# NVIDIA/audio-flamingo

Hardware: AMD Instinct MI355X
Metric: audio-sec/s + decoder tokens/s, AF3-7B bf16 train (higher is better)
Workload: dtype bf16; 1 GPU; AF3 (AF-Whisper 32L + Qwen2.5-7B 28L, MLP projector) bf16 train step fwd+bwd+AdamW, 30 s clips, S=1024; micro_batch_per_gpu=8, global_batch=8, seq_len=1024, parallelism=dp1, activation_checkpointing=False

## Files before the change

### audio-flamingo_amd/csrc/ceiling.hip

```cpp
#include "common.h"
#include "../../include/afk.h"

namespace {

constexpr int SEG = 16;

template <int MODE>
__global__ __launch_bounds__(512, 1) void mfma_ceiling_kernel(const bf16* __restrict__ src, float* __restrict__ sink, int iters) {
    extern __shared__ __attribute__((aligned(16))) char smem[];
    const int tid = threadIdx.x, lane = tid & 63, wave = tid >> 6;
    bf16x8 a[2][4], b[2][4];
    const bf16x8* s8 = (const bf16x8*)src;
#pragma unroll
    for (int i = 0; i < 2; ++i)
#pragma unroll
        for (int k = 0; k < 4; ++k) {
            a[i][k] = s8[((blockIdx.x * 8 + wave) * 16 + i * 4 + k) * 64 % 8192 + lane];
            b[i][k] = s8[((blockIdx.x * 8 + wave) * 16 + 8 + i * 4 + k) * 64 % 8192 + lane];
        }
    if (MODE == 1) {
        for (int i = tid; i < 4096; i += 512) ((bf16x8*)smem)[i] = s8[i];
        __syncthreads();
    }
    f32x16 acc[2][2];
#pragma unroll
    for (int i = 0; i < 2; ++i)
#pragma unroll
        for (int j = 0; j < 2; ++j)
#pragma unroll
            for (int e = 0; e < 16; ++e) acc[i][j][e] = 0.f;
    uint32_t lds = afk_lds_addr(smem) + lane * 16;
    for (int it = 0; it < iters; ++it) {
        if (MODE == 1) {
            const uint32_t base = lds + ((it * 12 * 1024) & 0xffff & ~0x3fff);
            afk_static_for<4>([&](auto K) {
                constexpr int k = decltype(K)::value;
                a[0][k] = afk_lds_b128<k * 1024>(base);
                a[1][k] = afk_lds_b128<(4 + k) * 1024>(base);
                b[k & 1][k] = afk_lds_b128<(8 + k) * 1024>(base);
            });
            afk_lds_wait0(a[0][0], a[0][1], a[0][2], a[0][3], a[1][0], a[1][1], a[1][2], a[1][3], b[0][0], b[1][1], b[0][2], b[1][3]);
        }
#pragma unroll
        for (int k = 0; k < 4; ++k)
#pragma unroll
            for (int i = 0; i < 2; ++i)
#pragma unroll
                for (int j = 0; j < 2; ++j) acc[i][j] = __builtin_amdgcn_mfma_f32_32x32x16_bf16(a[i][k], b[j][k], acc[i][j], 0, 0, 0);
    }
    float s = 0.f;
#pragma unroll
    for (int i = 0; i < 2; ++i)
#pragma unroll
        for (int j = 0; j < 2; ++j)
#pragma unroll
            for (int e = 0; e < 16; ++e) s += acc[i][j][e];
    if (s == 123.456f) sink[0] = s;
}

template <bool CHAIN>
__global__ __launch_bounds__(256, 1) void mfma_pacing_kernel(const bf16* __restrict__ src, float* __restrict__ sink, int iters) {
    const int lane = threadIdx.x & 63, wave = threadIdx.x >> 6;
    const bf16x8* s8 = (const bf16x8*)src;
    bf16x8 a[4], b[4];
#pragma unroll
    for (int k = 0; k < 4; ++k) {
        a[k] = s8[(wave * 8 + k) * 64 + lane];
        b[k] = s8[(wave * 8 + 4 + k) * 64 + lane];
    }
    f32x16 acc[4];
#pragma unroll
    for (int i = 0; i < 4; ++i)
#pragma unroll
        for (int e = 0; e < 16; ++e) acc[i][e] = 0.f;
    uint64_t t0, t1;
    asm volatile("s_waitcnt vmcnt(0)\n s_memtime %0\n s_waitcnt lgkmcnt(0)" : "=s"(t0)::"memory");
    for (int it = 0; it < iters; ++it) {
        if (CHAIN) {
#pragma unroll
            for (int i = 0; i < 4; ++i)
#pragma unroll
                for (int k = 0; k < 4; ++k) acc[i] = __builtin_amdgcn_mfma_f32_32x32x16_bf16(a[k], b[k], acc[i], 0, 0, 0);
        } else {
#pragma unroll
            for (int k = 0; k < 4; ++k)
#pragma unroll
                for (int i = 0; i < 4; ++i) acc[i] = __builtin_amdgcn_mfma_f32_32x32x16_bf16(a[k], b[k], acc[i], 0, 0, 0);
        }
    }
    float s = 0.f;
#pragma unroll
    for (int i = 0; i < 4; ++i)
#pragma unroll
        for (int e = 0; e < 16; ++e) s += acc[i][e];
    asm volatile("s_nop 0\n s_memtime %0\n s_waitcnt lgkmcnt(0)" : "=s"(t1) : "v"(s) : "memory");
    if (blockIdx.x == 0 && threadIdx.x == 0) sink[0] = (float)(t1 - t0) / (16.f * iters);
    if (s == 123.456f) sink[1] = s;
}

}

extern "C" int afk_mfma_ceiling(int mode, int nblocks, int iters, const void* operands, float* sink, double* host_flops, void* stream) {
    AFK_REQUIRE(mode >= 0 && mode <= 3, "afk_mfma_ceiling: mode %d (0 = register-resident operands, 1 = + LDS fragment reads, 2 / 3 = issue pacing of one wave per SIMD, "
                "independent / dependent accumulators: sink[0] = cycles per MFMA)", mode);
    AFK_REQUIRE(nblocks > 0 && iters > 0 && operands && sink, "afk_mfma_ceiling: bad arguments");
    hipStream_t s = (hipStream_t)stream;
    if (mode >= 2) {
        if (mode == 2) mfma_pacing_kernel<false><<<nblocks, 256, 0, s>>>((const bf16*)operands, sink, iters);
        else mfma_pacing_kernel<true><<<nblocks, 256, 0, s>>>((const bf16*)operands, sink, iters);
        AFK_LAUNCH_CHECK("afk_mfma_ceiling");
        if (host_flops) *host_flops = (double)nblocks * 4.0 * iters * 16 * 2.0 * 32 * 32 * 16;
        return AFK_OK;
    }
    if (mode == 0) {
        mfma_ceiling_kernel<0><<<nblocks, 512, 0, s>>>((const bf16*)operands, sink, iters);
    } else {
        static bool attr = false;
        if (!attr) {
            hipFuncSetAttribute((const void*)mfma_ceiling_kernel<1>, hipFuncAttributeMaxDynamicSharedMemorySize, 65536 + 16384);
            attr = true;
        }
        mfma_ceiling_kernel<1><<<nblocks, 512, 65536 + 16384, s>>>((const bf16*)operands, sink, iters);
    }
    AFK_LAUNCH_CHECK("afk_mfma_ceiling");
    if (host_flops) *host_flops = (double)nblocks * 8.0 * iters * SEG * 2.0 * 32 * 32 * 16;
    return AFK_OK;
}
```

### audio-flamingo_amd/csrc/gemm.hip

```cpp
#include "gemm_common.h"
#include <vector>
#include <mutex>

namespace {

constexpr int BM = 128, BN = 128, BK = 64;
constexpr int ROWB = BK * 2;
constexpr int STAGE_BYTES = (BM + BN) * ROWB;
constexpr int NSTAGE = 2;

__global__ __launch_bounds__(256, 2) void gemm_nt_bf16_k128(GemmArgs p) {
    extern __shared__ __attribute__((aligned(16))) char smem[];
    const int tid = threadIdx.x;
    const int lane = tid & 63;
    const int wave = __builtin_amdgcn_readfirstlane(tid >> 6);
    const int wm = wave >> 1, wn = wave & 1;
    const int hi = lane >> 5, l31 = lane & 31;

    int tm, tn;
    gemm_tile_of_block(p, tm, tn);
    const int m0 = tm * BM, n0 = tn * BN;

    const bf16* a_src[4];
    const bf16* b_src[4];
#pragma unroll
    for (int u = 0; u < 4; ++u) {
        const int unit = wave + 4 * u;
        const int rl = unit * 8 + (lane >> 3);
        const int chunk = (lane & 7) ^ ((rl >> 1) & 7);
        const int ra = min(m0 + rl, p.M - 1);
        const int rb = min(n0 + rl, p.N - 1);
        a_src[u] = p.A + (int64_t)ra * p.lda + chunk * 8;
        b_src[u] = p.B + (int64_t)rb * p.ldb + chunk * 8;
    }

    auto stage = [&](int buf, int kt) {
        char* sa = smem + buf * STAGE_BYTES;
        char* sb = sa + BM * ROWB;
        const int koff = kt * BK;
#pragma unroll
        for (int u = 0; u < 4; ++u) {
            const int unit = wave + 4 * u;
            __builtin_amdgcn_global_load_lds((gbl_void*)(a_src[u] + koff), (lds_void*)(sa + unit * 1024), 16, 0, 0);
        }
#pragma unroll
        for (int u = 0; u < 4; ++u) {
            const int unit = wave + 4 * u;
            __builtin_amdgcn_global_load_lds((gbl_void*)(b_src[u] + koff), (lds_void*)(sb + unit * 1024), 16, 0, 0);
        }
    };

    const int swz_l = (lane >> 1) & 7;
    int a_off[4], b_off[4];
#pragma unroll
    for (int s = 0; s < 4; ++s) {
        const int c = ((2 * s + hi) ^ swz_l) << 4;
        a_off[s] = (wm * 64 + l31) * ROWB + c;
        b_off[s] = (wn * 64 + l31) * ROWB + c;
    }

    f32x16 acc[2][2];
#pragma unroll
    for (int i = 0; i < 2; ++i)
#pragma unroll
        for (int j = 0; j < 2; ++j)
#pragma unroll
            for (int e = 0; e < 16; ++e) acc[i][j][e] = 0.f;

    int kt0 = 0, nkt = p.K / BK;
    if (p.splits > 1) {
        const int all = nkt, sp = blockIdx.y;
        kt0 = (int)((int64_t)all * sp / p.splits);
        nkt = (int)((int64_t)all * (sp + 1) / p.splits);
    }
    if (kt0 < nkt) stage(kt0 & 1, kt0);
    __syncthreads();
    for (int kt = kt0; kt < nkt; ++kt) {
        const int cur = kt & 1;
        if (kt + 1 < nkt) stage(cur ^ 1, kt + 1);
        const char* sa = smem + cur * STAGE_BYTES;
        const char* sb = sa + BM * ROWB;
#pragma unroll
        for (int s = 0; s < 4; ++s) {
            bf16x8 af[2], bfr[2];
#pragma unroll
            for (int i = 0; i < 2; ++i) af[i] = *(const bf16x8*)(sa + a_off[s] + i * 32 * ROWB);
#pragma unroll
            for (int j = 0; j < 2; ++j) bfr[j] = *(const bf16x8*)(sb + b_off[s] + j * 32 * ROWB);
#pragma unroll
            for (int i = 0; i < 2; ++i)
#pragma unroll
                for (int j = 0; j < 2; ++j)
                    acc[i][j] = __builtin_amdgcn_mfma_f32_32x32x16_bf16(bfr[j], af[i], acc[i][j], 0, 0, 0);
        }
        __syncthreads();
    }

#pragma unroll
    for (int i = 0; i < 2; ++i)
#pragma unroll
        for (int j = 0; j < 2; ++j) gemm_store_block32_body<-1>(p, m0 + wm * 64 + i * 32 + l31, n0 + wn * 64 + j * 32, hi, acc[i][j]);
}

#define AFK_GEMV_MAX_M 1
template <int MB, int R>
__global__ __launch_bounds__(256) void gemv_nt_bf16_kernel(GemmArgs p) {
    const int lane = threadIdx.x & 63, wave = threadIdx.x >> 6;
    const int n0 = (blockIdx.x * 4 + wave) * R;
    if (n0 >= p.N) return;
    const int kb_all = (p.K + 511) >> 9;
    const int kb0 = (int)((int64_t)kb_all * blockIdx.y / p.splits), kb1 = (int)((int64_t)kb_all * (blockIdx.y + 1) / p.splits);
    float acc[R][MB];
#pragma unroll
    for (int r = 0; r < R; ++r)
#pragma unroll
        for (int m = 0; m < MB; ++m) acc[r][m] = 0.f;
    const bf16* wrow[R];
#pragma unroll
    for (int r = 0; r < R; ++r) wrow[r] = p.B + (int64_t)min(n0 + r, p.N - 1) * p.ldb;
    for (int kb = kb0; kb < kb1; ++kb) {
        const int k = (kb << 9) + lane * 8;
        if (k < p.K) {
            bf16x8 wv[R], xv[MB];
#pragma unroll
            for (int r = 0; r < R; ++r) wv[r] = __builtin_nontemporal_load((const bf16x8*)(wrow[r] + k));
#pragma unroll
            for (int m = 0; m < MB; ++m) xv[m] = *(const bf16x8*)(p.A + (int64_t)min(m, p.M - 1) * p.lda + k);
#pragma unroll
            for (int r = 0; r < R; ++r)
#pragma unroll
                for (int m = 0; m < MB; ++m)
#pragma unroll
                    for (int e = 0; e < 4; ++e) {
                        const bf16x2 a = {wv[r][2 * e], wv[r][2 * e + 1]}, b = {xv[m][2 * e], xv[m][2 * e + 1]};
                        acc[r][m] = __builtin_amdgcn_fdot2_f32_bf16(a, b, acc[r][m], false);
                    }
        }
    }
    constexpr int V = R * MB;
    static_assert((V & (V - 1)) == 0 && V <= 64, "R*MB must be a power of two <= 64");
    float* v = &acc[0][0];
    int n = V;
#pragma unroll
    for (int sft = 5; sft >= 0; --sft) {
        const int st = 1 << sft;
        const bool up = (lane >> sft) & 1;
        if (n > 1) {
            const int h = n >> 1;
#pragma unroll
            for (int i = 0; i < V / 2; ++i)
                if (i < h) {
                    const float lo = v[i], hi_ = v[i + h];
                    v[i] = (up ? hi_ : lo) + __shfl_xor(up ? lo : hi_, st, 64);
                }
            n = h;
        } else {
            v[0] += __shfl_xor(v[0], st, 64);
        }
    }
    constexpr int LOGV = V == 64 ? 6 : V == 32 ? 5 : V == 16 ? 4 : V == 8 ? 3 : V == 4 ? 2 : V == 2 ? 1 : 0;
    const int idx = lane >> (6 - LOGV);
    const int r = idx / MB, m = idx % MB;
    if ((lane & ((64 >> LOGV) - 1)) == 0 && n0 + r < p.N && m < p.M) p.ws[((int64_t)blockIdx.y * p.M + m) * p.N + n0 + r] = v[0];
}

__global__ __launch_bounds__(256) void gemm_splitk_reduce_kernel(GemmArgs p) {
    const int n4 = p.N >> 2;
    const int64_t total = (int64_t)p.M * n4;
    for (int64_t t = (int64_t)blockIdx.x * blockDim.x + threadIdx.x; t < total; t += (int64_t)gridDim.x * blockDim.x) {
        const int m = (int)(t / n4), n = (int)(t % n4) * 4;
        const float* src = p.ws + (int64_t)m * p.N + n;
        f32x4 acc = *(const f32x4*)src;
        for (int sp = 1; sp < p.splits; ++sp) {
            const f32x4 x = *(const f32x4*)(src + (int64_t)sp * p.M * p.N);
#pragma unroll
            for (int e = 0; e < 4; ++e) acc[e] += x[e];
        }
        float v[4] = {acc[0], acc[1], acc[2], acc[3]};
        gemm_epilogue_store4(p, m, n, v);
    }
}

struct ProfState {
    std::mutex mu;
    bool on = false;
    std::vector<hipEvent_t> pool;
    size_t used = 0;
    double flops = 0.0;
    int64_t launches = 0;
    struct Rec { int M, N, K, variant; };
    std::vector<Rec> recs;
};
ProfState g_prof;
int g_variant = 0;
[[maybe_unused]] int g_256_impl = 2;
int g_gm = 0;
int g_wide = 1;

hipEvent_t prof_next_event() {
    if (g_prof.used == g_prof.pool.size()) {
        hipEvent_t e;
        hipEventCreate(&e);
        g_prof.pool.push_back(e);
    }
    return g_prof.pool[g_prof.used++];
}

}

extern "C" int afk_gemm_set_variant(int v) {
    const int gm = (v >> 8) & 255, base = v & 15;
#ifdef AFK_PROBES
    AFK_REQUIRE(base >= 0 && base <= 14, "afk_gemm_set_variant: 14 = persistent tile loop with the next tile's prologue issued ahead of the epilogue stores (round-4 probe), 13 = 256x256 ping-pong as a persistent tile loop, 0 auto, 1 = 128x128, 2 = 256x256 8-wave ping-pong, 3 = 256x256 4-wave (4, 5: its timing probes), 6 = 256x256 8-wave free-running BK=64 (7, 8, 9: probes), 10 = 8-wave free-running BK=32 ring-10 (11: probe)");
#else
    AFK_REQUIRE(base >= 0 && base <= 2, "afk_gemm_set_variant: variant %d is a probe / rejected schedule; this libafk.so was built without -DAFK_PROBES (make PROBES=1)", base);
    AFK_REQUIRE((gm & 0xc0) == 0, "afk_gemm_set_variant: gm bits 6 / 7 are timing probes (wrong results); this libafk.so was built without -DAFK_PROBES");
#endif
    g_gm = gm;
    g_wide = (v & 16) ? 0 : 1;
    g_variant = base;
    return AFK_OK;
}

extern "C" int afk_prof_enable(int on) {
    std::lock_guard<std::mutex> lk(g_prof.mu);
    g_prof.on = on != 0;
    return AFK_OK;
}

extern "C" int afk_prof_reset(void) {
    std::lock_guard<std::mutex> lk(g_prof.mu);
    g_prof.used = 0;
    g_prof.flops = 0.0;
    g_prof.launches = 0;
    g_prof.recs.clear();
    return AFK_OK;
}

extern "C" int afk_prof_collect(double* total_ms, double* total_flops, int64_t* launches) {
    std::lock_guard<std::mutex> lk(g_prof.mu);
    double ms = 0.0;
    for (size_t i = 0; i + 1 < g_prof.used; i += 2) {
        if (hipEventSynchronize(g_prof.pool[i + 1]) != hipSuccess)
            return afk_set_error(AFK_ERR_LAUNCH, "afk_prof_collect: event sync failed");
        float t = 0.f;
        if (hipEventElapsedTime(&t, g_prof.pool[i], g_prof.pool[i + 1]) != hipSuccess)
            return afk_set_error(AFK_ERR_LAUNCH, "afk_prof_collect: elapsed failed");
        ms += t;
    }
    if (total_ms) *total_ms = ms;
    if (total_flops) *total_flops = g_prof.flops;
    if (launches) *launches = g_prof.launches;
    return AFK_OK;
}

struct RopeEpi { const void *cos_t, *sin_t; const int* pos; int S, cols; const void *cos_lanes, *sin_lanes; };

static int gemm_impl(int trans_a, int trans_b, const void* A, int64_t lda, const void* B, int64_t ldb, void* C, int64_t ldc,
                     int M, int N, int K, const void* bias, const void* residual, int64_t ldr,
                     int res_mod, void* preact_out, float alpha, int flags, void* stream, int splits = 1, void* workspace = nullptr,
                     const RopeEpi* rope = nullptr) {
    AFK_REQUIRE(splits >= 1 && splits <= 64 && (splits == 1 || workspace), "afk_gemm_*_splitk: 1..64 splits, workspace required");
    AFK_REQUIRE(((flags & AFK_GEMM_ROPE) != 0) == (rope != nullptr), "afk_gemm: AFK_GEMM_ROPE belongs to afk_gemm_nt_bf16_rope");
    AFK_REQUIRE(splits == 1 || splits <= (K + BK - 1) / BK, "afk_gemm_*_splitk: more splits than K tiles");
    const bool gemv = workspace != nullptr && M <= AFK_GEMV_MAX_M && !trans_a && !trans_b;
    AFK_REQUIRE(!gemv || splits <= (K + 511) / 512, "afk_gemm_nt_bf16_splitk: M <= 16 streams K in blocks of 512: at most ceil(K/512) splits");
    AFK_REQUIRE(A && B && C, "afk_gemm_nt_bf16: null operand");
    AFK_REQUIRE(M > 0 && N > 0 && K > 0, "afk_gemm_nt_bf16: bad shape %d %d %d", M, N, K);
    AFK_REQUIRE(!trans_a || trans_b, "afk_gemm_bf16: A^T with k-contiguous B is not implemented (NT, NN, TN are)");
    AFK_REQUIRE(trans_a || K % BK == 0, "afk_gemm_nt_bf16: K=%d must be a multiple of %d (pad the operand)", K, BK);
    AFK_REQUIRE(!trans_b || (N % 8 == 0 && N >= 8), "afk_gemm_bf16: N=%d must be a multiple of 8 for a reduction-major B", N);
    AFK_REQUIRE(!trans_a || (M % 8 == 0 && M >= 8), "afk_gemm_bf16: M=%d must be a multiple of 8 for a reduction-major A", M);
    AFK_REQUIRE(N % 4 == 0, "afk_gemm_nt_bf16: N=%d must be a multiple of 4", N);
    AFK_REQUIRE(lda % 8 == 0 && ldb % 8 == 0 && ldc % 4 == 0, "afk_gemm_nt_bf16: leading dims must keep 16-B (A,B) / 8-B (C) alignment");
    AFK_REQUIRE(!(flags & AFK_GEMM_BIAS) || bias, "afk_gemm_nt_bf16: BIAS flag without bias");
    AFK_REQUIRE(!(flags & AFK_GEMM_RESIDUAL) || (residual && ldr % 4 == 0), "afk_gemm_nt_bf16: RESIDUAL flag without residual");
    AFK_REQUIRE(!(flags & AFK_GEMM_SWIGLU_FWD) || (flags == AFK_GEMM_SWIGLU_FWD && !trans_a && !trans_b && preact_out && N % 256 == 0 && splits == 1 &&
                                                     ldc % 8 == 0 && (uintptr_t)C % 16 == 0 && (uintptr_t)preact_out % 16 == 0),
                "afk_gemm_nt_bf16: SWIGLU_FWD needs the NT form, preact_out, N = 2I with I %% 128 == 0 and no other flag");
    AFK_REQUIRE(!(flags & AFK_GEMM_SWIGLU_BWD) || (residual && ldr % 4 == 0 && ldc >= 2 * (int64_t)N && flags == AFK_GEMM_SWIGLU_BWD && splits == 1),
                "afk_gemm: SWIGLU_BWD needs the gate|up tensor as `residual`, a [M, 2N] output and no other epilogue flag");
    AFK_REQUIRE(((uintptr_t)A % 16 == 0) && ((uintptr_t)B % 16 == 0) && ((uintptr_t)C % 8 == 0), "afk_gemm_nt_bf16: misaligned pointer");
    GemmArgs p;
    p.A = (const bf16*)A;
    p.B = (const bf16*)B;
    p.C = C;
    p.C2 = preact_out;
    p.bias = (const bf16*)bias;
    p.R = (const bf16*)residual;
    p.lda = lda;
    p.ldb = ldb;
    p.ldc = ldc;
    p.ldr = ldr;
    p.M = M;
    p.N = N;
    p.K = K;
    p.flags = flags;
    p.res_mod = res_mod;
    p.alpha = alpha;
    p.gm = g_gm;
    p.splits = splits;
    p.ws = (float*)workspace;
    p.rope_cos = rope ? (const bf16*)rope->cos_t : nullptr;
    p.rope_sin = rope ? (const bf16*)rope->sin_t : nullptr;
    p.rope_pos = rope ? rope->pos : nullptr;
    p.rope_S = rope ? rope->S : 1;
    p.rope_cols = rope ? rope->cols : 0;
    const bool lanes_ok = rope && rope->cos_lanes && rope->sin_lanes && !rope->pos && rope->S % 32 == 0;
    p.rope_cos_lanes = lanes_ok ? (const bf16*)rope->cos_lanes : nullptr;
    p.rope_sin_lanes = lanes_ok ? (const bf16*)rope->sin_lanes : nullptr;
    {
        const bool f32 = (flags & AFK_GEMM_OUT_F32) != 0;
        bool w = N % 8 == 0 && ldc % 8 == 0 && (uintptr_t)C % (f32 ? 32 : 16) == 0;
        if (flags & AFK_GEMM_BIAS) w = w && (uintptr_t)bias % 16 == 0;
        if (flags & (AFK_GEMM_RESIDUAL | AFK_GEMM_SWIGLU_BWD)) w = w && ldr % 8 == 0 && (uintptr_t)residual % 16 == 0;
        if (preact_out) w = w && (uintptr_t)preact_out % 16 == 0;
        p.wide = w && g_wide ? 1 : 0;
    }
    const int64_t tiles256 = afk_cdiv(M, 256) * afk_cdiv(N, 256);
    const bool use256 = !gemv && (trans_b || (flags & AFK_GEMM_SWIGLU_FWD) || (splits == 1 && (g_variant >= 2 || (g_variant == 0 && tiles256 >= 192))));
    if (rope && (!use256 || !p.wide || trans_a || trans_b || splits != 1))
        return afk_set_error(AFK_ERR_UNSUPPORTED, "afk_gemm_nt_bf16_rope: needs the 256 x 256 NT kernel (>= 192 tiles) in its 16-byte epilogue form; use "
                                                  "afk_gemm_nt_bf16 + afk_rope_inplace for this shape");
#ifdef AFK_PROBES
    static const int env_impl = [] {
        const char* e = getenv("AFK_GEMM256");
        return (e && e[0] == 'p' && e[1] == 'e') ? 13 : (e && e[0] == 'p') ? 2 : (e && e[0] == 'w') ? 3 : (e && e[0] == 'f') ? 10 : 0;
    }();
    const int impl256 = (flags & (AFK_GEMM_SWIGLU_FWD | AFK_GEMM_ROPE)) ? 2 : g_variant >= 2 ? g_variant : (env_impl ? env_impl : g_256_impl);
    const bool w4 = use256 && !trans_b && impl256 >= 3 && impl256 <= 9;
    const bool f8 = use256 && !trans_b && impl256 >= 10 && impl256 <= 12;
    const bool persist = use256 && !trans_b && impl256 == 13;
    const bool persist_q = use256 && !trans_b && impl256 == 14;
#endif
    if ((flags & AFK_GEMM_SWIGLU_FWD) && !p.wide)
        return afk_set_error(AFK_ERR_UNSUPPORTED, "afk_gemm_nt_bf16: SWIGLU_FWD needs the 16-byte epilogue form (aligned C / preact_out, ldc %% 8 == 0, "
                                                  "afk_gemm_set_variant bit 4 clear)");
    p.ntm = (int)afk_cdiv(M, use256 ? 256 : BM);
    p.ntn = (int)afk_cdiv(N, use256 ? 256 : BN);
    static bool attr_set = false;
    if (!attr_set) {
        hipFuncSetAttribute((const void*)gemm_nt_bf16_k128, hipFuncAttributeMaxDynamicSharedMemorySize, NSTAGE * STAGE_BYTES);
        attr_set = true;
    }
    hipStream_t st = (hipStream_t)stream;
    const int64_t nwg = (int64_t)p.ntm * p.ntn;
    AFK_REQUIRE(nwg < (1ll << 31), "afk_gemm_nt_bf16: grid too large");
    hipEvent_t e0 = nullptr, e1 = nullptr;
    bool prof = false;
    {
        std::lock_guard<std::mutex> lk(g_prof.mu);
        prof = g_prof.on;
        if (prof) {
            e0 = prof_next_event();
            e1 = prof_next_event();
            g_prof.flops += 2.0 * (double)M * (double)N * (double)K;
            g_prof.launches += 1;
            g_prof.recs.push_back({M, N, K, trans_b ? (trans_a ? 4 : 3) : (use256 ? 2 : 1)});
        }
    }
    afk_count(gemv ? AFK_CNT_GEMV : trans_b ? (trans_a ? AFK_CNT_GEMM_TN256 : AFK_CNT_GEMM_NN256) : use256 ? AFK_CNT_GEMM_NT256 : AFK_CNT_GEMM_NT128);
    if (splits > 1) afk_count(AFK_CNT_GEMM_SPLITK);
    if (prof) hipEventRecord(e0, st);
    if (gemv) {
        const dim3 grid((unsigned)afk_cdiv(N, 32), (unsigned)splits);
#define AFK_GEMV(MB_, R_) hipLaunchKernelGGL((gemv_nt_bf16_kernel<MB_, R_>), grid, dim3(256), 0, st, p)
        AFK_GEMV(1, 8);
#undef AFK_GEMV
        int g = (int)afk_cdiv((int64_t)M * (N / 4), 256);
        if (g > 2048) g = 2048;
        hipLaunchKernelGGL(gemm_splitk_reduce_kernel, dim3(g), dim3(256), 0, st, p);
    } else if (trans_b) {
        if (int e = afk_launch_gemm256t(p, trans_a, st)) return e;
        if (splits > 1) {
            int g = (int)afk_cdiv((int64_t)M * (N / 4), 256);
            if (g > 2048) g = 2048;
            hipLaunchKernelGGL(gemm_splitk_reduce_kernel, dim3(g), dim3(256), 0, st, p);
        }
    } else if (use256) {
#ifdef AFK_PROBES
        if (int e = persist_q ? afk_launch_gemm256q(p, st) : persist ? afk_launch_gemm256p(p, st) : f8 ? afk_launch_gemm256f8(p, impl256 - 10, st) : w4 ? afk_launch_gemm256w4(p, impl256 - 3, st) : afk_launch_gemm256(p, st)) return e;
#else
        if (int e = afk_launch_gemm256(p, st)) return e;
#endif
    } else {
        hipLaunchKernelGGL(gemm_nt_bf16_k128, dim3((unsigned)nwg, (unsigned)splits), dim3(256), NSTAGE * STAGE_BYTES, st, p);
        if (splits > 1) {
            int g = (int)afk_cdiv((int64_t)M * (N / 4), 256);
            if (g > 2048) g = 2048;
            hipLaunchKernelGGL(gemm_splitk_reduce_kernel, dim3(g), dim3(256), 0, st, p);
        }
    }
    if (prof) hipEventRecord(e1, st);
    AFK_LAUNCH_CHECK("afk_gemm_nt_bf16");
    return AFK_OK;
}

extern "C" int afk_gemm_nt_bf16(const void* A, int64_t lda, const void* B, int64_t ldb, void* C, int64_t ldc,
                                int M, int N, int K, const void* bias, const void* residual, int64_t ldr,
                                int res_mod, void* preact_out, float alpha, int flags, void* stream) {
    return gemm_impl(0, 0, A, lda, B, ldb, C, ldc, M, N, K, bias, residual, ldr, res_mod, preact_out, alpha, flags, stream);
}

extern "C" int afk_gemm_nt_bf16_rope(const void* A, int64_t lda, const void* B, int64_t ldb, void* C, int64_t ldc, int M, int N, int K, const void* bias,
                                     const void* cos_t, const void* sin_t, const int* pos, int S, int rope_cols, const void* cos_lanes, const void* sin_lanes,
                                     void* stream) {
    AFK_REQUIRE(cos_t && sin_t && (uintptr_t)cos_t % 16 == 0 && (uintptr_t)sin_t % 16 == 0, "afk_gemm_nt_bf16_rope: cos / sin tables (16-byte aligned) are required");
    AFK_REQUIRE(N % 256 == 0 && rope_cols >= 0 && rope_cols <= N && rope_cols % 256 == 0 && S > 0,
                "afk_gemm_nt_bf16_rope: N and rope_cols must be multiples of 256 (two 128-column heads per tile), S > 0");
    AFK_REQUIRE((cos_lanes == nullptr) == (sin_lanes == nullptr) && (!cos_lanes || ((uintptr_t)cos_lanes % 16 == 0 && (uintptr_t)sin_lanes % 16 == 0)),
                "afk_gemm_nt_bf16_rope: the lane-major tables come as a 16-byte aligned pair");
    const RopeEpi r = {cos_t, sin_t, pos, S, rope_cols, cos_lanes, sin_lanes};
    return gemm_impl(0, 0, A, lda, B, ldb, C, ldc, M, N, K, bias, nullptr, 0, 0, nullptr, 1.f, AFK_GEMM_ROPE | (bias ? AFK_GEMM_BIAS : 0), stream, 1, nullptr, &r);
}

extern "C" int afk_gemm_nt_bf16_splitk(const void* A, int64_t lda, const void* B, int64_t ldb, void* C, int64_t ldc, int M, int N, int K,
                                       const void* bias, const void* residual, int64_t ldr, int res_mod, void* preact_out, float alpha,
                                       int flags, int splits, void* workspace, void* stream) {
    return gemm_impl(0, 0, A, lda, B, ldb, C, ldc, M, N, K, bias, residual, ldr, res_mod, preact_out, alpha, flags, stream, splits, workspace);
}

extern "C" int afk_gemv_partials(const void* A, int64_t lda, const void* B, int64_t ldb, int M, int N, int K, int splits, float* workspace,
                                 void* stream) {
    AFK_REQUIRE(A && B && workspace && M >= 1 && M <= AFK_GEMV_MAX_M && N > 0 && K > 0 && K % 8 == 0 && lda % 8 == 0 && ldb % 8 == 0,
                "afk_gemv_partials: bad args (M <= %d, K %% 8 == 0)", AFK_GEMV_MAX_M);
    AFK_REQUIRE(splits >= 1 && splits <= (K + 511) / 512 && splits <= 64, "afk_gemv_partials: 1 <= splits <= ceil(K / 512)");
    GemmArgs p = {};
    p.A = (const bf16*)A; p.B = (const bf16*)B; p.lda = lda; p.ldb = ldb; p.M = M; p.N = N; p.K = K; p.splits = splits; p.ws = workspace;
    const dim3 grid((unsigned)afk_cdiv(N, 32), (unsigned)splits);
    hipStream_t st = (hipStream_t)stream;
    hipLaunchKernelGGL((gemv_nt_bf16_kernel<1, 8>), grid, dim3(256), 0, st, p);
    AFK_LAUNCH_CHECK("afk_gemv_partials");
    return AFK_OK;
}

extern "C" int afk_gemm_bf16_splitk(int trans_a, int trans_b, const void* A, int64_t lda, const void* B, int64_t ldb, void* C, int64_t ldc,
                                    int M, int N, int K, const void* bias, const void* residual, int64_t ldr, int res_mod, void* preact_out,
                                    float alpha, int flags, int splits, void* workspace, void* stream) {
    return gemm_impl(trans_a, trans_b, A, lda, B, ldb, C, ldc, M, N, K, bias, residual, ldr, res_mod, preact_out, alpha, flags, stream, splits,
                     workspace);
}

extern "C" int afk_gemm_bf16(int trans_a, int trans_b, const void* A, int64_t lda, const void* B, int64_t ldb, void* C,
                             int64_t ldc, int M, int N, int K, const void* bias, const void* residual, int64_t ldr,
                             int res_mod, void* preact_out, float alpha, int flags, void* stream) {
    return gemm_impl(trans_a, trans_b, A, lda, B, ldb, C, ldc, M, N, K, bias, residual, ldr, res_mod, preact_out, alpha, flags, stream);
}

extern "C" int afk_prof_dump(const char* host_path) {
    std::lock_guard<std::mutex> lk(g_prof.mu);
    FILE* f = fopen(host_path, "w");
    if (!f) return afk_set_error(AFK_ERR_ARG, "afk_prof_dump: cannot open %s", host_path);
    fprintf(f, "M,N,K,variant,ms\n");
    for (size_t i = 0; i < g_prof.recs.size() && 2 * i + 1 < g_prof.used; ++i) {
        float ms = 0.f;
        hipEventSynchronize(g_prof.pool[2 * i + 1]);
        hipEventElapsedTime(&ms, g_prof.pool[2 * i], g_prof.pool[2 * i + 1]);
        fprintf(f, "%d,%d,%d,%d,%.6f\n", g_prof.recs[i].M, g_prof.recs[i].N, g_prof.recs[i].K, g_prof.recs[i].variant, ms);
    }
    fclose(f);
    return AFK_OK;
}
```

### audio-flamingo_amd/csrc/gemm256.hip

```cpp
#include "gemm_common.h"

namespace {

constexpr int BM = 256, BN = 256, BK = 64;
constexpr int ROWB = 128;
constexpr int OP_BYTES = 256 * ROWB;
constexpr int BUF_BYTES = 2 * OP_BYTES;
constexpr int LDS_BYTES = 2 * BUF_BYTES;

#define AFK_VMCNT(n) asm volatile("s_waitcnt vmcnt(" #n ")" ::: "memory")
#define AFK_LGKMCNT0() asm volatile("s_waitcnt lgkmcnt(0)" ::: "memory")
#define AFK_BARRIER()                         \
    do {                                      \
        __builtin_amdgcn_sched_barrier(0);    \
        __builtin_amdgcn_s_barrier();         \
        __builtin_amdgcn_sched_barrier(0);    \
    } while (0)

template <int EPI>
__global__ __launch_bounds__(512, 1) void gemm_nt_bf16_k256(GemmArgs p) {
    extern __shared__ __attribute__((aligned(16))) char smem[];
    const int tid = threadIdx.x;
    const int lane = tid & 63;
    const int wave = __builtin_amdgcn_readfirstlane(tid >> 6);
    const int wm = wave >> 2, wn = wave & 3;
    const int hi = lane >> 5, l31 = lane & 31;

    int tm, tn;
    gemm_tile_of_block(p, tm, tn);
    const int m0 = tm * BM, n0 = tn * BN;

    const bf16* xsrc[6];
    int xdst[6];
    const bf16* ysrc[2];
    int ydst[2];
    {
        const int lrow = lane >> 3, pos = lane & 7;
#pragma unroll
        for (int j = 0; j < 6; ++j) {
            const int i = wave + 8 * j;
            const bool isB = i < 32;
            const int unit = isB ? i : ((i - 32) < 8 ? (i - 32) : (i - 32) + 8);
            const int rl = unit * 8 + lrow;
            const int chunk = pos ^ ((rl >> 1) & 7);
            if (isB) {
                const int r = (EPI == AFK_GEMM_SWIGLU_FWD) ? (rl < 128 ? tn * 128 + rl : (p.N >> 1) + tn * 128 + rl - 128) : min(n0 + rl, p.N - 1);
                xsrc[j] = p.B + (int64_t)r * p.ldb + chunk * 8;
            } else {
                const int r = min(m0 + rl, p.M - 1);
                xsrc[j] = p.A + (int64_t)r * p.lda + chunk * 8;
            }
            xdst[j] = (isB ? OP_BYTES : 0) + unit * 1024;
        }
#pragma unroll
        for (int j = 0; j < 2; ++j) {
            const int jj = wave + 8 * j;
            const int unit = jj < 8 ? 8 + jj : 16 + jj;
            const int rl = unit * 8 + lrow;
            const int chunk = pos ^ ((rl >> 1) & 7);
            const int r = min(m0 + rl, p.M - 1);
            ysrc[j] = p.A + (int64_t)r * p.lda + chunk * 8;
            ydst[j] = unit * 1024;
        }
    }
    auto issue_x = [&](int t) {
        char* base = smem + (t & 1) * BUF_BYTES;
        const int koff = t * BK;
#pragma unroll
        for (int j = 0; j < 6; ++j)
            __builtin_amdgcn_global_load_lds((gbl_void*)(xsrc[j] + koff), (lds_void*)(base + xdst[j]), 16, 0, 0);
    };
    auto issue_y = [&](int t) {
        char* base = smem + (t & 1) * BUF_BYTES;
        const int koff = t * BK;
#pragma unroll
        for (int j = 0; j < 2; ++j)
            __builtin_amdgcn_global_load_lds((gbl_void*)(ysrc[j] + koff), (lds_void*)(base + ydst[j]), 16, 0, 0);
    };

    const int swz_l = (lane >> 1) & 7;
    int koffb[4];
#pragma unroll
    for (int s = 0; s < 4; ++s) koffb[s] = ((2 * s + hi) ^ swz_l) << 4;
    const int a_row0 = (wm * 128 + l31) * ROWB;
    const int b_row0 = OP_BYTES + (wn * 64 + l31) * ROWB;

    f32x16 acc[4][2];
#pragma unroll
    for (int i = 0; i < 4; ++i)
#pragma unroll
        for (int j = 0; j < 2; ++j)
#pragma unroll
            for (int e = 0; e < 16; ++e) acc[i][j][e] = 0.f;

    const int T = p.K / BK;
    issue_x(0);
    issue_y(0);
    if (T > 1) {
        issue_x(1);
        AFK_VMCNT(8);
    } else {
        AFK_VMCNT(2);
    }
    AFK_BARRIER();
    if (wm == 1) AFK_BARRIER();

    bf16x8 bf[2][4], af[2][4];
#define AFK_MFMA4(ACC0, s)                                                                                         \
    do {                                                                                                           \
        _Pragma("unroll") for (int i_ = 0; i_ < 2; ++i_) _Pragma("unroll") for (int j_ = 0; j_ < 2; ++j_)          \
            acc[ACC0 + i_][j_] = __builtin_amdgcn_mfma_f32_32x32x16_bf16(bf[j_][s], af[i_][s], acc[ACC0 + i_][j_], 0, 0, 0); \
    } while (0)
    for (int t = 0; t < T; ++t) {
        const char* buf = smem + (t & 1) * BUF_BYTES;
        const int t1 = min(t + 1, T - 1), t2 = min(t + 2, T - 1);
        const int e1 = (t + 1) & 1, e2 = t & 1;
        const int64_t oy = (int64_t)t1 * BK, ox = (int64_t)t2 * BK;
        char* by = smem + e1 * BUF_BYTES;
        char* bx = smem + e2 * BUF_BYTES;
#pragma unroll
        for (int j = 0; j < 2; ++j)
#pragma unroll
            for (int s = 0; s < 4; ++s) bf[j][s] = *(const bf16x8*)(buf + b_row0 + j * 32 * ROWB + koffb[s]);
#pragma unroll
        for (int i = 0; i < 2; ++i)
#pragma unroll
            for (int s = 0; s < 4; ++s) af[i][s] = *(const bf16x8*)(buf + a_row0 + i * 32 * ROWB + koffb[s]);
        AFK_LGKMCNT0();
        AFK_VMCNT(6);
        AFK_BARRIER();
        __builtin_amdgcn_s_setprio(1);
        AFK_MFMA4(0, 0);
        __builtin_amdgcn_sched_barrier(0);
        __builtin_amdgcn_global_load_lds((gbl_void*)(ysrc[0] + oy), (lds_void*)(by + ydst[0]), 16, 0, 0);
        __builtin_amdgcn_sched_barrier(0);
        AFK_MFMA4(0, 1);
        __builtin_amdgcn_sched_barrier(0);
        __builtin_amdgcn_global_load_lds((gbl_void*)(ysrc[1] + oy), (lds_void*)(by + ydst[1]), 16, 0, 0);
        __builtin_amdgcn_sched_barrier(0);
        AFK_MFMA4(0, 2);
        AFK_MFMA4(0, 3);
        __builtin_amdgcn_s_setprio(0);
        AFK_VMCNT(8);
        AFK_BARRIER();
#pragma unroll
        for (int i = 0; i < 2; ++i)
#pragma unroll
            for (int s = 0; s < 4; ++s) af[i][s] = *(const bf16x8*)(buf + a_row0 + (i + 2) * 32 * ROWB + koffb[s]);
        AFK_LGKMCNT0();
        AFK_VMCNT(2);
        AFK_BARRIER();
        __builtin_amdgcn_s_setprio(1);
#pragma unroll
        for (int s = 0; s < 4; ++s) {
#pragma unroll
            for (int i = 0; i < 2; ++i) {
                acc[2 + i][0] = __builtin_amdgcn_mfma_f32_32x32x16_bf16(bf[0][s], af[i][s], acc[2 + i][0], 0, 0, 0);
                acc[2 + i][1] = __builtin_amdgcn_mfma_f32_32x32x16_bf16(bf[1][s], af[i][s], acc[2 + i][1], 0, 0, 0);
                const int piece = 2 * s + i;
                if (piece < 6) {
                    __builtin_amdgcn_sched_barrier(0);
                    __builtin_amdgcn_global_load_lds((gbl_void*)(xsrc[piece] + ox), (lds_void*)(bx + xdst[piece]), 16, 0, 0);
                    __builtin_amdgcn_sched_barrier(0);
                }
            }
        }
        __builtin_amdgcn_s_setprio(0);
        AFK_VMCNT(8);
        AFK_BARRIER();
    }
    AFK_VMCNT(0);
#undef AFK_MFMA4
    if (wm == 0) AFK_BARRIER();

    if constexpr (EPI == AFK_GEMM_SWIGLU_FWD) {
        typedef __attribute__((ext_vector_type(8))) __bf16 b8;
        const int I = p.N >> 1;
        const bool up = wn >= 2;
        const int feat0 = tn * 128 + (wn & 1) * 64;
        char* xch = smem + (wm * 2 + (wn & 1)) * 16384 + lane * 16;
        b8 pc[16];
#pragma unroll
        for (int i = 0; i < 4; ++i)
#pragma unroll
            for (int j = 0; j < 2; ++j)
#pragma unroll
                for (int t = 0; t < 2; ++t) {
                    b8 o;
#pragma unroll
                    for (int e = 0; e < 4; ++e) {
                        const auto r = __builtin_amdgcn_permlane32_swap(__float_as_uint(acc[i][j][8 * t + e]), __float_as_uint(acc[i][j][8 * t + 4 + e]), false, false);
                        o[e] = (bf16)(__uint_as_float(r[0]) * p.alpha);
                        o[4 + e] = (bf16)(__uint_as_float(r[1]) * p.alpha);
                    }
                    pc[(i * 2 + j) * 2 + t] = o;
                }
        if (up) {
#pragma unroll
            for (int q = 0; q < 16; ++q) *(b8*)(xch + q * 1024) = pc[q];
        }
        __syncthreads();
#pragma unroll
        for (int i = 0; i < 4; ++i) {
            const int m = m0 + wm * 128 + i * 32 + l31;
#pragma unroll
            for (int j = 0; j < 2; ++j)
#pragma unroll
                for (int t = 0; t < 2; ++t) {
                    const int q = (i * 2 + j) * 2 + t;
                    const int f = feat0 + j * 32 + 16 * t + 8 * hi;
                    if (!up) {
                        const b8 u = *(const b8*)(xch + q * 1024);
                        b8 h;
#pragma unroll
                        for (int e = 0; e < 8; ++e) {
                            const float gf = (float)pc[q][e];
                            h[e] = (bf16)(rbf(gf * sigmoid_f(gf)) * (float)u[e]);
                        }
                        if (m < p.M) *(b8*)((bf16*)p.C2 + (int64_t)m * I + f) = h;
                    }
                    if (m < p.M) *(b8*)((bf16*)p.C + (int64_t)m * p.ldc + (up ? I : 0) + f) = pc[q];
                }
        }
        return;
    }
    if constexpr (EPI >= 0 && (EPI & AFK_GEMM_ROPE) != 0) {
        typedef __attribute__((ext_vector_type(8))) __bf16 b8;
        const bool rot = n0 < p.rope_cols;
        char* mine = smem + (wm * 4 + wn) * 16384 + lane * 16;
        const char* theirs = smem + (wm * 4 + (wn ^ 1)) * 16384 + lane * 16;
        b8 pc[16];
#pragma unroll
        for (int i = 0; i < 4; ++i)
#pragma unroll
            for (int j = 0; j < 2; ++j)
#pragma unroll
                for (int t = 0; t < 2; ++t) {
                    const int n = n0 + wn * 64 + j * 32 + 16 * t + 8 * hi;
                    b8 bv;
                    if constexpr ((EPI & AFK_GEMM_BIAS) != 0) bv = *(const b8*)(p.bias + n);
                    b8 o;
#pragma unroll
                    for (int e = 0; e < 4; ++e) {
                        const auto r = __builtin_amdgcn_permlane32_swap(__float_as_uint(acc[i][j][8 * t + e]), __float_as_uint(acc[i][j][8 * t + 4 + e]), false, false);
                        float v0 = __uint_as_float(r[0]) * p.alpha, v1 = __uint_as_float(r[1]) * p.alpha;
                        if constexpr ((EPI & AFK_GEMM_BIAS) != 0) {
                            v0 += (float)bv[e];
                            v1 += (float)bv[4 + e];
                        }
                        o[e] = (bf16)v0;
                        o[4 + e] = (bf16)v1;
                    }
                    pc[(i * 2 + j) * 2 + t] = o;
                }
        if (rot) {
#pragma unroll
            for (int q = 0; q < 16; ++q) *(b8*)(mine + q * 1024) = pc[q];
        }
        __syncthreads();
#pragma unroll
        for (int i = 0; i < 4; ++i) {
            const int m = m0 + wm * 128 + i * 32 + l31;
            const int mc = min(m, p.M - 1);
            const int64_t pr = p.rope_pos ? p.rope_pos[mc] : mc % p.rope_S;
            const bool lanes = p.rope_cos_lanes != nullptr;
            const int64_t lbase = lanes ? (((int64_t)((m0 + wm * 128 + i * 32) % p.rope_S) >> 5) * 16 * 32 + l31) * 8 : 0;
#pragma unroll
            for (int j = 0; j < 2; ++j)
#pragma unroll
                for (int t = 0; t < 2; ++t) {
                    const int q = (i * 2 + j) * 2 + t;
                    const int cl = wn * 64 + j * 32 + 16 * t + 8 * hi;
                    b8 o = pc[q];
                    if (rot) {
                        const int d = cl & 127;
                        const b8 other = *(const b8*)(theirs + q * 1024);
                        const b8 c = lanes ? *(const b8*)(p.rope_cos_lanes + lbase + (d >> 3) * 256) : *(const b8*)(p.rope_cos + pr * 128 + d);
                        const b8 sn = lanes ? *(const b8*)(p.rope_sin_lanes + lbase + (d >> 3) * 256) : *(const b8*)(p.rope_sin + pr * 128 + d);
                        const float sg = (wn & 1) ? 1.f : -1.f;
#pragma unroll
                        for (int e = 0; e < 8; ++e)
                            o[e] = (bf16)(rbf_strict((float)pc[q][e] * (float)c[e]) + rbf_strict(sg * (float)other[e] * (float)sn[e]));
                    }
                    if (m < p.M) *(b8*)((bf16*)p.C + (int64_t)m * p.ldc + n0 + cl) = o;
                }
        }
        return;
    }
    if (AFK_GM_NOEPI(p)) return;
#pragma unroll
    for (int i = 0; i < 4; ++i)
#pragma unroll
        for (int j = 0; j < 2; ++j) gemm_store_block32<EPI>(p, m0 + wm * 128 + i * 32 + l31, n0 + wn * 64 + j * 32, hi, acc[i][j]);
}

}

#define AFK_EPI_LIST(X) X(0) X(AFK_GEMM_BIAS) X(AFK_GEMM_RESIDUAL) X(AFK_GEMM_BIAS | AFK_GEMM_RESIDUAL) X(AFK_GEMM_BIAS | AFK_GEMM_GELU) \
    X(AFK_GEMM_BIAS | AFK_GEMM_GELU | AFK_GEMM_RESIDUAL) X(AFK_GEMM_ACCUM) X(AFK_GEMM_SWIGLU_FWD) X(AFK_GEMM_SWIGLU_BWD) X(AFK_GEMM_ROPE) X(AFK_GEMM_ROPE | AFK_GEMM_BIAS) X(-1)

int afk_launch_gemm256(const GemmArgs& p, hipStream_t st) {
    static bool attr_set = false;
    if (!attr_set) {
#define AFK_SET(F)                                                                                                                       \
    if (hipFuncSetAttribute((const void*)gemm_nt_bf16_k256<(F)>, hipFuncAttributeMaxDynamicSharedMemorySize, LDS_BYTES) != hipSuccess) \
        return afk_set_error(AFK_ERR_LAUNCH, "gemm256: cannot reserve %d bytes of LDS", LDS_BYTES);
        AFK_EPI_LIST(AFK_SET)
#undef AFK_SET
        attr_set = true;
    }
    const int64_t nwg = (int64_t)p.ntm * p.ntn;
    const int f = (p.wide && p.splits <= 1) ? p.flags : -1;
    switch (f) {
#define AFK_CASE(F)                                                                                          \
    case (F):                                                                                                \
        if ((F) == -1) afk_count(AFK_CNT_GEMM_GENERIC);                                                      \
        hipLaunchKernelGGL(gemm_nt_bf16_k256<(F)>, dim3((unsigned)nwg), dim3(512), LDS_BYTES, st, p);        \
        break;
        AFK_EPI_LIST(AFK_CASE)
#undef AFK_CASE
        default:
            afk_count(AFK_CNT_GEMM_GENERIC);
            hipLaunchKernelGGL(gemm_nt_bf16_k256<-1>, dim3((unsigned)nwg), dim3(512), LDS_BYTES, st, p);
    }
    return AFK_OK;
}
```

### audio-flamingo_amd/csrc/gemm256t.hip

```cpp
#include "gemm_common.h"

namespace {

constexpr int BK = 64;
constexpr int OP_BYTES = 32768;
constexpr int BUF_BYTES = 2 * OP_BYTES;
constexpr int LDS_BYTES = 2 * BUF_BYTES;
constexpr int TROW = 512;

typedef __attribute__((address_space(3))) bf16x4 lds_bf16x4;

#define AFK_VMCNT(n) asm volatile("s_waitcnt vmcnt(" #n ")" ::: "memory")
#define AFK_LGKMCNT0() asm volatile("s_waitcnt lgkmcnt(0)" ::: "memory")
#define AFK_BARRIER()                         \
    do {                                      \
        __builtin_amdgcn_sched_barrier(0);    \
        __builtin_amdgcn_s_barrier();         \
        __builtin_amdgcn_sched_barrier(0);    \
    } while (0)
#define AFK_DMA_PTR(SRCPTR, DSTPTR)                                                                       \
    do {                                                                                                  \
        __builtin_amdgcn_sched_barrier(0);                                                                \
        __builtin_amdgcn_global_load_lds((gbl_void*)(SRCPTR), (lds_void*)(DSTPTR), 16, 0, 0);             \
        __builtin_amdgcn_sched_barrier(0);                                                                \
    } while (0)
#define MFMA(a, b, c) __builtin_amdgcn_mfma_f32_32x32x16_bf16(a, b, c, 0, 0, 0)

__device__ __forceinline__ int tswz(int r) { return ((r & 3) << 2) | ((r >> 2) & 3); }

__device__ __forceinline__ int tr_off(int tile32, int pc, int lane) {
    const int g = lane >> 4, i = lane & 15, hi = g >> 1;
    const int chunk = 4 * tile32 + 2 * (g & 1) + ((i & 3) >> 1);
    const int r = 8 * hi + (i >> 2) + 4 * pc;
    return r * TROW + ((chunk ^ tswz(r)) << 4) + 8 * (i & 1);
}
template <int S>
__device__ __forceinline__ bf16x8 tr_frag(uint32_t buf, int off0, int off1) {
    return afk_lds_tr_frag<S * 16 * TROW>(buf + off0, buf + off1);
}

struct TSrc {
    const bf16* base;
    int krow;
};
__device__ __forceinline__ TSrc tsrc(const bf16* mat, int unit, int col0, int ncols, int lane) {
    const int krow = 2 * unit + (lane >> 5);
    const int pos = lane & 31;
    const int chunk = pos ^ tswz(krow);
    const int col = min(col0 + chunk * 8, ncols - 8);
    TSrc s;
    s.base = mat + col;
    s.krow = krow;
    return s;
}

template <bool AT, int EPI>
__global__ __launch_bounds__(512, 1) void gemm_xt_bf16_k256(GemmArgs p) {
    extern __shared__ __attribute__((aligned(16))) char smem[];
    const int tid = threadIdx.x;
    const int lane = tid & 63;
    const int wave = __builtin_amdgcn_readfirstlane(tid >> 6);
    const int wm = wave >> 2, wn = wave & 3;
    const int hi = lane >> 5, l31 = lane & 31;

    int tm, tn;
    gemm_tile_of_block(p, tm, tn);
    const int m0 = tm * 256, n0 = tn * 256;
    int KL = p.K;
    const bf16* Abase = p.A;
    const bf16* Bbase = p.B;
    if (p.splits > 1) {
        const int tall = (p.K + BK - 1) / BK;
        const int t0 = (int)((int64_t)tall * blockIdx.y / p.splits), t1 = (int)((int64_t)tall * (blockIdx.y + 1) / p.splits);
        const int kbeg = t0 * BK;
        KL = min(p.K, t1 * BK) - kbeg;
        Abase += AT ? (int64_t)kbeg * p.lda : (int64_t)kbeg;
        Bbase += (int64_t)kbeg * p.ldb;
    }
    const int T = (KL + BK - 1) / BK;
    constexpr int NX = AT ? 4 : 6, NY = AT ? 4 : 2;

    const bf16* an_src[NX + NY];
    TSrc tr_src[NX + NY];
    int64_t tr_ld[NX + NY];
    int dst[NX + NY];
#pragma unroll
    for (int j = 0; j < NX + NY; ++j) {
        const bool isx = j < NX;
        const int jj = isx ? j : j - NX;
        an_src[j] = nullptr;
        tr_src[j].base = nullptr;
        tr_src[j].krow = 0;
        tr_ld[j] = 0;
        if (AT) {
            const bool isA = jj < 2;
            const int unit = (isx ? 0 : 16) + wave + 8 * (jj & 1);
            tr_src[j] = isA ? tsrc(Abase, unit, m0, p.M, lane) : tsrc(Bbase, unit, n0, p.N, lane);
            tr_ld[j] = isA ? p.lda : p.ldb;
            dst[j] = (isA ? 0 : OP_BYTES) + unit * 1024;
        } else if (isx && jj < 4) {
            const int unit = wave + 8 * jj;
            tr_src[j] = tsrc(Bbase, unit, n0, p.N, lane);
            tr_ld[j] = p.ldb;
            dst[j] = OP_BYTES + unit * 1024;
        } else {
            const int k = wave + 8 * (isx ? jj - 4 : jj);
            const int unit = isx ? (k < 8 ? k : k + 8) : (k < 8 ? 8 + k : 16 + k);
            const int rl = unit * 8 + (lane >> 3);
            const int chunk = (lane & 7) ^ ((rl >> 1) & 7);
            const int r = min(m0 + rl, p.M - 1);
            an_src[j] = Abase + (int64_t)r * p.lda + chunk * 8;
            dst[j] = unit * 1024;
        }
    }
    const bf16* tbase[NX + NY];
#pragma unroll
    for (int j = 0; j < NX + NY; ++j) tbase[j] = (AT || j < 4) ? tr_src[j].base + (int64_t)tr_src[j].krow * tr_ld[j] : nullptr;
    f32x16 acc[4][2];
#pragma unroll
    for (int i = 0; i < 4; ++i)
#pragma unroll
        for (int j = 0; j < 2; ++j)
#pragma unroll
            for (int e = 0; e < 16; ++e) acc[i][j][e] = 0.f;

    const bool ragged = (KL % BK) != 0;
  auto pipeline = [&](auto rag_) {
    constexpr bool RAG = decltype(rag_)::value;
    auto src_of = [&](int j, int t) -> const bf16* {
        const bool tr = AT || j < 4;
        if (tr) {
            if constexpr (RAG) {
                const int row = min(t * BK + tr_src[j].krow, KL - 1);
                return tr_src[j].base + (int64_t)row * tr_ld[j];
            } else {
                return tbase[j] + (int64_t)t * BK * tr_ld[j];
            }
        }
        return an_src[j] + (int64_t)t * BK;
    };
    auto issue = [&](int j, int t_src, int parity) { AFK_DMA_PTR(src_of(j, t_src), smem + parity * BUF_BYTES + dst[j]); };

    int tob[2][2], toa[4][2];
#pragma unroll
    for (int j = 0; j < 2; ++j)
#pragma unroll
        for (int pc = 0; pc < 2; ++pc) tob[j][pc] = OP_BYTES + tr_off(wn * 2 + j, pc, lane);
#pragma unroll
    for (int i = 0; i < 4; ++i)
#pragma unroll
        for (int pc = 0; pc < 2; ++pc) toa[i][pc] = AT ? tr_off(wm * 4 + i, pc, lane) : 0;
    const int swz_l = (lane >> 1) & 7;
    int koffb[4];
#pragma unroll
    for (int s = 0; s < 4; ++s) koffb[s] = ((2 * s + hi) ^ swz_l) << 4;
    const int a_row0 = (wm * 128 + l31) * 128;

#pragma unroll
    for (int j = 0; j < NX; ++j) issue(j, 0, 0);
#pragma unroll
    for (int j = 0; j < NY; ++j) issue(NX + j, 0, 0);
    {
        const int t1 = min(1, T - 1);
#pragma unroll
        for (int j = 0; j < NX; ++j) issue(j, t1, 1);
    }
    if (AT) AFK_VMCNT(8); else AFK_VMCNT(8);
    AFK_BARRIER();
    if (wm == 1) AFK_BARRIER();

    bf16x8 bf[2][4], af[AT ? 4 : 2][AT ? 2 : 4];
    const uint32_t lds0 = afk_lds_addr(smem);
    for (int t = 0; t < T; ++t) {
        const char* buf = smem + (t & 1) * BUF_BYTES;
        const uint32_t lbuf = lds0 + (t & 1) * BUF_BYTES;
        const int t1 = min(t + 1, T - 1), t2 = min(t + 2, T - 1);
        const int e1 = (t + 1) & 1, e2 = t & 1;
        if (!AT) {
#pragma unroll
            for (int j = 0; j < 2; ++j)
                afk_static_for<4>([&](auto s_) { constexpr int s = decltype(s_)::value; bf[j][s] = tr_frag<s>(lbuf, tob[j][0], tob[j][1]); });
#pragma unroll
            for (int i = 0; i < 2; ++i)
#pragma unroll
                for (int s = 0; s < 4; ++s) af[i][s] = *(const bf16x8*)(buf + a_row0 + i * 32 * 128 + koffb[s]);
            AFK_LGKMCNT0();
            AFK_VMCNT(6);
            AFK_BARRIER();
            __builtin_amdgcn_s_setprio(1);
#pragma unroll
            for (int s = 0; s < 4; ++s) {
#pragma unroll
                for (int i = 0; i < 2; ++i)
#pragma unroll
                    for (int j = 0; j < 2; ++j) acc[i][j] = MFMA(bf[j][s], af[i][s], acc[i][j]);
                if (s < 2) issue(NX + s, t1, e1);
            }
            __builtin_amdgcn_s_setprio(0);
            AFK_VMCNT(8);
            AFK_BARRIER();
#pragma unroll
            for (int i = 0; i < 2; ++i)
#pragma unroll
                for (int s = 0; s < 4; ++s) af[i][s] = *(const bf16x8*)(buf + a_row0 + (i + 2) * 32 * 128 + koffb[s]);
            AFK_LGKMCNT0();
            AFK_VMCNT(2);
            AFK_BARRIER();
            __builtin_amdgcn_s_setprio(1);
#pragma unroll
            for (int s = 0; s < 4; ++s) {
#pragma unroll
                for (int i = 0; i < 2; ++i) {
                    acc[2 + i][0] = MFMA(bf[0][s], af[i][s], acc[2 + i][0]);
                    acc[2 + i][1] = MFMA(bf[1][s], af[i][s], acc[2 + i][1]);
                    const int piece = 2 * s + i;
                    if (piece < 6) issue(piece, t2, e2);
                }
            }
            __builtin_amdgcn_s_setprio(0);
            AFK_VMCNT(8);
            AFK_BARRIER();
        } else {
            const int kvalid = KL - t * BK;
#pragma unroll
            for (int ph = 0; ph < 2; ++ph) {
                afk_static_for<2>([&](auto s_) {
                    constexpr int s = decltype(s_)::value;
                    if (ph == 0) {
#pragma unroll
                        for (int j = 0; j < 2; ++j) bf[j][s] = tr_frag<s>(lbuf, tob[j][0], tob[j][1]);
#pragma unroll
                        for (int i = 0; i < 4; ++i) af[i][s] = tr_frag<s>(lbuf, toa[i][0], toa[i][1]);
                    } else {
#pragma unroll
                        for (int j = 0; j < 2; ++j) bf[j][s] = tr_frag<2 + s>(lbuf, tob[j][0], tob[j][1]);
#pragma unroll
                        for (int i = 0; i < 4; ++i) af[i][s] = tr_frag<2 + s>(lbuf, toa[i][0], toa[i][1]);
                    }
                });
                AFK_LGKMCNT0();
                if (RAG && kvalid < BK) {
#pragma unroll
                    for (int s = 0; s < 2; ++s)
#pragma unroll
                        for (int e = 0; e < 8; ++e) {
                            const bool dead = 16 * (2 * ph + s) + 8 * hi + e >= kvalid;
#pragma unroll
                            for (int i = 0; i < 4; ++i)
                                if (dead) af[i][s][e] = (bf16)0.f;
                        }
                }
                AFK_VMCNT(4);
                AFK_BARRIER();
                __builtin_amdgcn_s_setprio(1);
#pragma unroll
                for (int s = 0; s < 2; ++s) {
#pragma unroll
                    for (int i = 0; i < 4; ++i) {
                        acc[i][0] = MFMA(bf[0][s], af[i][s], acc[i][0]);
                        acc[i][1] = MFMA(bf[1][s], af[i][s], acc[i][1]);
                        const int piece = 4 * s + i;
                        if ((piece & 1) == 0) {
                            if (ph == 0) issue(NX + (piece >> 1), t1, e1);
                            else issue(piece >> 1, t2, e2);
                        }
                    }
                }
                __builtin_amdgcn_s_setprio(0);
                AFK_VMCNT(8);
                AFK_BARRIER();
            }
        }
    }
    AFK_VMCNT(0);
    if (wm == 0) AFK_BARRIER();
  };
    if (ragged) pipeline(std::true_type{});
    else pipeline(std::false_type{});

#pragma unroll
    for (int i = 0; i < 4; ++i)
#pragma unroll
        for (int j = 0; j < 2; ++j) gemm_store_block32<EPI>(p, m0 + wm * 128 + i * 32 + l31, n0 + wn * 64 + j * 32, hi, acc[i][j]);
}

}

#define AFK_EPI_LIST(X) X(0) X(AFK_GEMM_ACCUM) X(-2) X(-1)

int afk_launch_gemm256t(const GemmArgs& p, int trans_a, hipStream_t st) {
    static bool attr_set = false;
    if (!attr_set) {
#define AFK_SET(F)                                                                                                                                \
    if (hipFuncSetAttribute((const void*)gemm_xt_bf16_k256<false, (F)>, hipFuncAttributeMaxDynamicSharedMemorySize, LDS_BYTES) != hipSuccess || \
        hipFuncSetAttribute((const void*)gemm_xt_bf16_k256<true, (F)>, hipFuncAttributeMaxDynamicSharedMemorySize, LDS_BYTES) != hipSuccess)    \
        return afk_set_error(AFK_ERR_LAUNCH, "gemm256t: cannot reserve %d bytes of LDS", LDS_BYTES);
        AFK_EPI_LIST(AFK_SET)
#undef AFK_SET
        attr_set = true;
    }
    const int64_t nwg = (int64_t)p.ntm * p.ntn;
    const unsigned ns = (unsigned)(p.splits > 1 ? p.splits : 1);
    const int f = p.splits > 1 ? -2 : (p.wide ? p.flags : -1);
    const dim3 grid((unsigned)nwg, ns);
    switch (f) {
#define AFK_CASE(F)                                                                                                   \
    case (F):                                                                                                         \
        if ((F) == -1) afk_count(AFK_CNT_GEMM_GENERIC);                                                               \
        if (trans_a) hipLaunchKernelGGL((gemm_xt_bf16_k256<true, (F)>), grid, dim3(512), LDS_BYTES, st, p);          \
        else hipLaunchKernelGGL((gemm_xt_bf16_k256<false, (F)>), grid, dim3(512), LDS_BYTES, st, p);                 \
        break;
        AFK_EPI_LIST(AFK_CASE)
#undef AFK_CASE
        default:
            afk_count(AFK_CNT_GEMM_GENERIC);
            if (trans_a) hipLaunchKernelGGL((gemm_xt_bf16_k256<true, -1>), grid, dim3(512), LDS_BYTES, st, p);
            else hipLaunchKernelGGL((gemm_xt_bf16_k256<false, -1>), grid, dim3(512), LDS_BYTES, st, p);
    }
    return AFK_OK;
}
```

### audio-flamingo_amd/csrc/gemm_common.h

```cpp
#pragma once
#include "common.h"
#include "../../include/afk.h"

struct GemmArgs {
    const bf16* A;
    const bf16* B;
    void* C;
    void* C2;
    const bf16* bias;
    const bf16* R;
    int64_t lda, ldb, ldc, ldr;
    int M, N, K;
    int ntm, ntn;
    int flags;
    int res_mod;
    float alpha;
    int gm;
    int splits;
    float* ws;
    int wide;
    const bf16* rope_cos;
    const bf16* rope_sin;
    const int* rope_pos;
    int rope_S, rope_cols;
    const bf16* rope_cos_lanes;
    const bf16* rope_sin_lanes;
};

#ifdef AFK_PROBES
#define AFK_GM_NOEPI(p) (((p).gm & 0x40) != 0)
#define AFK_GM_RAW(p) (((p).gm & 0x80) != 0)
#else
#define AFK_GM_NOEPI(p) false
#define AFK_GM_RAW(p) false
#endif

typedef __attribute__((address_space(3))) void lds_void;
typedef const __attribute__((address_space(1))) void gbl_void;

__device__ __forceinline__ void gemm_tile_of(const GemmArgs& p, int bid, int nwg, int& tm, int& tn) {
    const int xcd = bid & 7, idx = bid >> 3, q = nwg >> 3, r = nwg & 7;
    const int swz = AFK_GM_RAW(p) ? bid : (xcd < r ? xcd * (q + 1) : r * (q + 1) + (xcd - r) * q) + idx;
    const int GM = (p.gm & 0x3f) > 0 ? (p.gm & 0x3f) : 4;
    const int per_group = GM * p.ntn;
    const int g = swz / per_group, rem = swz - g * per_group;
    const int first_m = g * GM;
    const int gsz = min(p.ntm - first_m, GM);
    tm = first_m + rem % gsz;
    tn = rem / gsz;
}
__device__ __forceinline__ void gemm_tile_of_block(const GemmArgs& p, int& tm, int& tn) { gemm_tile_of(p, blockIdx.x, gridDim.x, tm, tn); }

template <int W, int F = -1>
__device__ __forceinline__ void gemm_epilogue_store(const GemmArgs& p, int m, int n, float* v) {
    typedef __attribute__((ext_vector_type(W))) __bf16 bvec;
    typedef __attribute__((ext_vector_type(W))) float fvec;
    const int flags = F >= 0 ? F : p.flags;
#pragma unroll
    for (int e = 0; e < W; ++e) v[e] *= p.alpha;
    if (flags & AFK_GEMM_BIAS) {
        const bvec bv = *(const bvec*)(p.bias + n);
#pragma unroll
        for (int e = 0; e < W; ++e) v[e] += (float)bv[e];
    }
    if (flags & AFK_GEMM_GELU) {
#pragma unroll
        for (int e = 0; e < W; ++e) v[e] = rbf(v[e]);
        if (p.C2) {
            bvec pre;
#pragma unroll
            for (int e = 0; e < W; ++e) pre[e] = (bf16)v[e];
            *(bvec*)((bf16*)p.C2 + (int64_t)m * p.ldc + n) = pre;
        }
#pragma unroll
        for (int e = 0; e < W; ++e) v[e] = gelu_f(v[e]);
    }
    if (flags & AFK_GEMM_SWIGLU_BWD) {
        const bvec gv = *(const bvec*)(p.R + (int64_t)m * p.ldr + n);
        const bvec uv = *(const bvec*)(p.R + (int64_t)m * p.ldr + p.N + n);
        bvec og, ou;
#pragma unroll
        for (int e = 0; e < W; ++e) {
            const float gf = (float)gv[e], uf = (float)uv[e], df = rbf(v[e]);
            const float s = sigmoid_f(gf);
            og[e] = (bf16)(df * uf * (s * (1.f + gf * (1.f - s))));
            ou[e] = (bf16)(df * (gf * s));
        }
        bf16* cp = (bf16*)p.C + (int64_t)m * p.ldc + n;
        *(bvec*)cp = og;
        *(bvec*)(cp + p.N) = ou;
        return;
    }
    if (flags & AFK_GEMM_RESIDUAL) {
        const int rm = p.res_mod > 0 ? m % p.res_mod : m;
        const bvec rv = *(const bvec*)(p.R + (int64_t)rm * p.ldr + n);
#pragma unroll
        for (int e = 0; e < W; ++e) v[e] = rbf(v[e]) + (float)rv[e];
    }
    if (flags & AFK_GEMM_OUT_F32) {
        float* cp = (float*)p.C + (int64_t)m * p.ldc + n;
        fvec o;
        if (flags & AFK_GEMM_ACCUM) {
            o = *(const fvec*)cp;
#pragma unroll
            for (int e = 0; e < W; ++e) o[e] += v[e];
        } else {
#pragma unroll
            for (int e = 0; e < W; ++e) o[e] = v[e];
        }
        *(fvec*)cp = o;
    } else {
        bf16* cp = (bf16*)p.C + (int64_t)m * p.ldc + n;
        if (flags & AFK_GEMM_ACCUM) {
            const bvec old = *(const bvec*)cp;
#pragma unroll
            for (int e = 0; e < W; ++e) v[e] += (float)old[e];
        }
        bvec o;
#pragma unroll
        for (int e = 0; e < W; ++e) o[e] = (bf16)v[e];
        *(bvec*)cp = o;
    }
}
__device__ __forceinline__ void gemm_epilogue_store4(const GemmArgs& p, int m, int n, float v[4]) { gemm_epilogue_store<4, -1>(p, m, n, v); }

template <int F>
__device__ __forceinline__ void gemm_store_block32_body(const GemmArgs& p, int m, int nb, int hi, const f32x16& acc);
static __device__ __noinline__ void gemm_store_block32_generic(const GemmArgs& p, int m, int nb, int hi, f32x16 acc) {
    gemm_store_block32_body<-1>(p, m, nb, hi, acc);
}
template <int F = -1>
__device__ __forceinline__ void gemm_store_block32(const GemmArgs& p, int m, int nb, int hi, const f32x16& acc) {
    if constexpr (F == -1) gemm_store_block32_generic(p, m, nb, hi, acc);
    else gemm_store_block32_body<F>(p, m, nb, hi, acc);
}
template <int F>
__device__ __forceinline__ void gemm_store_block32_body(const GemmArgs& p, int m, int nb, int hi, const f32x16& acc) {
    if (m >= p.M) return;
    if (F == -2 || (F == -1 && p.splits > 1)) {
#pragma unroll
        for (int q = 0; q < 4; ++q) {
            const int n = nb + 8 * q + 4 * hi;
            if (n >= p.N) continue;
            const f32x4 o = {acc[4 * q], acc[4 * q + 1], acc[4 * q + 2], acc[4 * q + 3]};
            *(f32x4*)(p.ws + ((int64_t)blockIdx.y * p.M + m) * p.N + n) = o;
        }
        return;
    }
    if constexpr (F == -2) return;
    if (F >= 0 || p.wide) {
#pragma unroll
        for (int t = 0; t < 2; ++t) {
            float v[8];
#pragma unroll
            for (int e = 0; e < 4; ++e) {
                const auto r = __builtin_amdgcn_permlane32_swap(__float_as_uint(acc[8 * t + e]), __float_as_uint(acc[8 * t + 4 + e]), false, false);
                v[e] = __uint_as_float(r[0]);
                v[4 + e] = __uint_as_float(r[1]);
            }
            const int n = nb + 16 * t + 8 * hi;
            if (n < p.N) gemm_epilogue_store<8, F>(p, m, n, v);
        }
        return;
    }
#pragma unroll
    for (int q = 0; q < 4; ++q) {
        const int n = nb + 8 * q + 4 * hi;
        if (n >= p.N) continue;
        float v[4] = {acc[4 * q], acc[4 * q + 1], acc[4 * q + 2], acc[4 * q + 3]};
        gemm_epilogue_store<4, F>(p, m, n, v);
    }
}

int afk_launch_gemm256(const GemmArgs& p, hipStream_t st);
int afk_launch_gemm256p(const GemmArgs& p, hipStream_t st);
int afk_launch_gemm256q(const GemmArgs& p, hipStream_t st);
int afk_launch_gemm256f8(const GemmArgs& p, int mode, hipStream_t st);
int afk_launch_gemm256w4(const GemmArgs& p, int mode, hipStream_t st);
int afk_launch_gemm256t(const GemmArgs& p, int trans_a, hipStream_t st);
```

Measured before the change: 633.4 audio-s/s.

## Switch GEMM kernels to 16x16x32 bf16 MFMA tiles by default

Adds a compile-time path that builds the 128 and 256 tile GEMM kernels on v_mfma_f32_16x16x32_bf16 instead of 32x32x16. It reshapes accumulator arrays, LDS fragment offsets, DMA interleave points and epilogue gathers (permlane16_swap) to match, and makes it the default unless AFK_MFMA_32 is defined. A matching 16x16 MFMA ceiling microbenchmark mode is also added. The aim is higher MFMA throughput or better issue behaviour on MI355X. In exchange it needs more accumulator and fragment registers and more LDS reads per tile, plus a new epilogue layout that could carry correctness risk.

```diff
diff --git a/audio-flamingo_amd/csrc/ceiling.hip b/audio-flamingo_amd/csrc/ceiling.hip
--- a/audio-flamingo_amd/csrc/ceiling.hip
+++ b/audio-flamingo_amd/csrc/ceiling.hip
@@ -58,6 +58,59 @@
     if (s == 123.456f) sink[0] = s;
 }
 
+template <int MODE>
+__global__ __launch_bounds__(512, 1) void mfma_ceiling16_kernel(const bf16* __restrict__ src, float* __restrict__ sink, int iters) {
+    extern __shared__ __attribute__((aligned(16))) char smem[];
+    const int tid = threadIdx.x, lane = tid & 63, wave = tid >> 6;
+    bf16x8 a[4][2], b[4][2];
+    const bf16x8* s8 = (const bf16x8*)src;
+#pragma unroll
+    for (int i = 0; i < 4; ++i)
+#pragma unroll
+        for (int k = 0; k < 2; ++k) {
+            a[i][k] = s8[((blockIdx.x * 8 + wave) * 16 + i * 2 + k) * 64 % 8192 + lane];
+            b[i][k] = s8[((blockIdx.x * 8 + wave) * 16 + 8 + i * 2 + k) * 64 % 8192 + lane];
+        }
+    if (MODE == 1) {
+        for (int i = tid; i < 4096; i += 512) ((bf16x8*)smem)[i] = s8[i];
+        __syncthreads();
+    }
+    f32x4 acc[4][4];
+#pragma unroll
+    for (int i = 0; i < 4; ++i)
+#pragma unroll
+        for (int j = 0; j < 4; ++j)
+#pragma unroll
+            for (int e = 0; e < 4; ++e) acc[i][j][e] = 0.f;
+    uint32_t lds = afk_lds_addr(smem) + lane * 16;
+    for (int it = 0; it < iters; ++it) {
+        if (MODE == 1) {
+            const uint32_t base = lds + ((it * 12 * 1024) & 0xffff & ~0x3fff);
+            afk_static_for<4>([&](auto I) {
+                constexpr int i = decltype(I)::value;
+                a[i][0] = afk_lds_b128<(2 * i) * 1024>(base);
+                a[i][1] = afk_lds_b128<(2 * i + 1) * 1024>(base);
+                b[i][i & 1] = afk_lds_b128<(8 + i) * 1024>(base);
+            });
+            afk_lds_wait0(a[0][0], a[0][1], a[1][0], a[1][1], a[2][0], a[2][1], a[3][0], a[3][1], b[0][0], b[1][1], b[2][0], b[3][1]);
+        }
+#pragma unroll
+        for (int k = 0; k < 2; ++k)
+#pragma unroll
+            for (int i = 0; i < 4; ++i)
+#pragma unroll
+                for (int j = 0; j < 4; ++j) acc[i][j] = __builtin_amdgcn_mfma_f32_16x16x32_bf16(a[i][k], b[j][k], acc[i][j], 0, 0, 0);
+    }
+    float s = 0.f;
+#pragma unroll
+    for (int i = 0; i < 4; ++i)
+#pragma unroll
+        for (int j = 0; j < 4; ++j)
+#pragma unroll
+            for (int e = 0; e < 4; ++e) s += acc[i][j][e];
+    if (s == 123.456f) sink[0] = s;
+}
+
 template <bool CHAIN>
 __global__ __launch_bounds__(256, 1) void mfma_pacing_kernel(const bf16* __restrict__ src, float* __restrict__ sink, int iters) {
     const int lane = threadIdx.x & 63, wave = threadIdx.x >> 6;
@@ -101,11 +154,11 @@
 }
 
 extern "C" int afk_mfma_ceiling(int mode, int nblocks, int iters, const void* operands, float* sink, double* host_flops, void* stream) {
-    AFK_REQUIRE(mode >= 0 && mode <= 3, "afk_mfma_ceiling: mode %d (0 = register-resident operands, 1 = + LDS fragment reads, 2 / 3 = issue pacing of one wave per SIMD, "
-                "independent / dependent accumulators: sink[0] = cycles per MFMA)", mode);
+    AFK_REQUIRE(mode >= 0 && mode <= 5, "afk_mfma_ceiling: mode %d (0 = register-resident operands, 1 = + LDS fragment reads, 2 / 3 = issue pacing of one wave per SIMD, "
+                "independent / dependent accumulators: sink[0] = cycles per MFMA, 4 / 5 = modes 0 / 1 on v_mfma_f32_16x16x32_bf16)", mode);
     AFK_REQUIRE(nblocks > 0 && iters > 0 && operands && sink, "afk_mfma_ceiling: bad arguments");
     hipStream_t s = (hipStream_t)stream;
-    if (mode >= 2) {
+    if (mode == 2 || mode == 3) {
         if (mode == 2) mfma_pacing_kernel<false><<<nblocks, 256, 0, s>>>((const bf16*)operands, sink, iters);
         else mfma_pacing_kernel<true><<<nblocks, 256, 0, s>>>((const bf16*)operands, sink, iters);
         AFK_LAUNCH_CHECK("afk_mfma_ceiling");
@@ -114,6 +167,15 @@
     }
     if (mode == 0) {
         mfma_ceiling_kernel<0><<<nblocks, 512, 0, s>>>((const bf16*)operands, sink, iters);
+    } else if (mode == 4) {
+        mfma_ceiling16_kernel<0><<<nblocks, 512, 0, s>>>((const bf16*)operands, sink, iters);
+    } else if (mode == 5) {
+        static bool attr16 = false;
+        if (!attr16) {
+            hipFuncSetAttribute((const void*)mfma_ceiling16_kernel<1>, hipFuncAttributeMaxDynamicSharedMemorySize, 65536 + 16384);
+            attr16 = true;
+        }
+        mfma_ceiling16_kernel<1><<<nblocks, 512, 65536 + 16384, s>>>((const bf16*)operands, sink, iters);
     } else {
         static bool attr = false;
         if (!attr) {
@@ -123,6 +185,6 @@
         mfma_ceiling_kernel<1><<<nblocks, 512, 65536 + 16384, s>>>((const bf16*)operands, sink, iters);
     }
     AFK_LAUNCH_CHECK("afk_mfma_ceiling");
-    if (host_flops) *host_flops = (double)nblocks * 8.0 * iters * SEG * 2.0 * 32 * 32 * 16;
+    if (host_flops) *host_flops = mode >= 4 ? (double)nblocks * 8.0 * iters * (2 * SEG) * 2.0 * 16 * 16 * 32 : (double)nblocks * 8.0 * iters * SEG * 2.0 * 32 * 32 * 16;
     return AFK_OK;
 }
diff --git a/audio-flamingo_amd/csrc/gemm.hip b/audio-flamingo_amd/csrc/gemm.hip
--- a/audio-flamingo_amd/csrc/gemm.hip
+++ b/audio-flamingo_amd/csrc/gemm.hip
@@ -8,6 +8,15 @@
 constexpr int ROWB = BK * 2;
 constexpr int STAGE_BYTES = (BM + BN) * ROWB;
 constexpr int NSTAGE = 2;
+#ifdef AFK_MFMA_16
+constexpr int TR = 16, NT = 4, NS = 2;
+typedef f32x4 acc_t;
+#define AFK_MFMA(a, b, c) __builtin_amdgcn_mfma_f32_16x16x32_bf16(a, b, c, 0, 0, 0)
+#else
+constexpr int TR = 32, NT = 2, NS = 4;
+typedef f32x16 acc_t;
+#define AFK_MFMA(a, b, c) __builtin_amdgcn_mfma_f32_32x32x16_bf16(a, b, c, 0, 0, 0)
+#endif
 
 __global__ __launch_bounds__(256, 2) void gemm_nt_bf16_k128(GemmArgs p) {
     extern __shared__ __attribute__((aligned(16))) char smem[];
@@ -15,7 +24,7 @@
     const int lane = tid & 63;
     const int wave = __builtin_amdgcn_readfirstlane(tid >> 6);
     const int wm = wave >> 1, wn = wave & 1;
-    const int hi = lane >> 5, l31 = lane & 31;
+    [[maybe_unused]] const int hi = lane >> 5, l31 = lane & 31;
 
     int tm, tn;
     gemm_tile_of_block(p, tm, tn);
@@ -51,21 +60,22 @@
     };
 
     const int swz_l = (lane >> 1) & 7;
-    int a_off[4], b_off[4];
-#pragma unroll
-    for (int s = 0; s < 4; ++s) {
-        const int c = ((2 * s + hi) ^ swz_l) << 4;
-        a_off[s] = (wm * 64 + l31) * ROWB + c;
-        b_off[s] = (wn * 64 + l31) * ROWB + c;
-    }
-
-    f32x16 acc[2][2];
-#pragma unroll
-    for (int i = 0; i < 2; ++i)
-#pragma unroll
-        for (int j = 0; j < 2; ++j)
-#pragma unroll
-            for (int e = 0; e < 16; ++e) acc[i][j][e] = 0.f;
+    const int lrow = lane & (TR - 1), lk = lane / TR;
+    int a_off[NS], b_off[NS];
+#pragma unroll
+    for (int s = 0; s < NS; ++s) {
+        const int c = (((8 / NS) * s + lk) ^ swz_l) << 4;
+        a_off[s] = (wm * 64 + lrow) * ROWB + c;
+        b_off[s] = (wn * 64 + lrow) * ROWB + c;
+    }
+
+    acc_t acc[NT][NT];
+#pragma unroll
+    for (int i = 0; i < NT; ++i)
+#pragma unroll
+        for (int j = 0; j < NT; ++j)
+#pragma unroll
+            for (int e = 0; e < TR * TR / 64; ++e) acc[i][j][e] = 0.f;
 
     int kt0 = 0, nkt = p.K / BK;
     if (p.splits > 1) {
@@ -81,17 +91,16 @@
         const char* sa = smem + cur * STAGE_BYTES;
         const char* sb = sa + BM * ROWB;
 #pragma unroll
-        for (int s = 0; s < 4; ++s) {
-            bf16x8 af[2], bfr[2];
-#pragma unroll
-            for (int i = 0; i < 2; ++i) af[i] = *(const bf16x8*)(sa + a_off[s] + i * 32 * ROWB);
-#pragma unroll
-            for (int j = 0; j < 2; ++j) bfr[j] = *(const bf16x8*)(sb + b_off[s] + j * 32 * ROWB);
-#pragma unroll
-            for (int i = 0; i < 2; ++i)
-#pragma unroll
-                for (int j = 0; j < 2; ++j)
-                    acc[i][j] = __builtin_amdgcn_mfma_f32_32x32x16_bf16(bfr[j], af[i], acc[i][j], 0, 0, 0);
+        for (int s = 0; s < NS; ++s) {
+            bf16x8 af[NT], bfr[NT];
+#pragma unroll
+            for (int i = 0; i < NT; ++i) af[i] = *(const bf16x8*)(sa + a_off[s] + i * TR * ROWB);
+#pragma unroll
+            for (int j = 0; j < NT; ++j) bfr[j] = *(const bf16x8*)(sb + b_off[s] + j * TR * ROWB);
+#pragma unroll
+            for (int i = 0; i < NT; ++i)
+#pragma unroll
+                for (int j = 0; j < NT; ++j) acc[i][j] = AFK_MFMA(bfr[j], af[i], acc[i][j]);
         }
         __syncthreads();
     }
@@ -99,7 +108,14 @@
 #pragma unroll
     for (int i = 0; i < 2; ++i)
 #pragma unroll
-        for (int j = 0; j < 2; ++j) gemm_store_block32_body<-1>(p, m0 + wm * 64 + i * 32 + l31, n0 + wn * 64 + j * 32, hi, acc[i][j]);
+        for (int j = 0; j < 2; ++j) {
+#ifdef AFK_MFMA_16
+            const GemmBlock16 blk = {{acc[2 * i][2 * j], acc[2 * i][2 * j + 1], acc[2 * i + 1][2 * j], acc[2 * i + 1][2 * j + 1]}};
+            gemm_store_block16_body<-1>(p, m0 + wm * 64 + i * 32, n0 + wn * 64 + j * 32, lane, blk);
+#else
+            gemm_store_block32_body<-1>(p, m0 + wm * 64 + i * 32 + l31, n0 + wn * 64 + j * 32, hi, acc[i][j]);
+#endif
+        }
 }
 
 #define AFK_GEMV_MAX_M 1
diff --git a/audio-flamingo_amd/csrc/gemm256.hip b/audio-flamingo_amd/csrc/gemm256.hip
--- a/audio-flamingo_amd/csrc/gemm256.hip
+++ b/audio-flamingo_amd/csrc/gemm256.hip
@@ -7,6 +7,18 @@
 constexpr int OP_BYTES = 256 * ROWB;
 constexpr int BUF_BYTES = 2 * OP_BYTES;
 constexpr int LDS_BYTES = 2 * BUF_BYTES;
+
+#ifdef AFK_MFMA_16
+constexpr int TR = 16, NI = 8, NJ = 4, NS = 2;
+typedef f32x4 acc_t;
+#define AFK_MFMA(a, b, c) __builtin_amdgcn_mfma_f32_16x16x32_bf16(a, b, c, 0, 0, 0)
+#else
+constexpr int TR = 32, NI = 4, NJ = 2, NS = 4;
+typedef f32x16 acc_t;
+#define AFK_MFMA(a, b, c) __builtin_amdgcn_mfma_f32_32x32x16_bf16(a, b, c, 0, 0, 0)
+#endif
+constexpr int NE = TR * TR / 64;
+constexpr int QSEG = (NI / 2) * NJ * NS / 4;
 
 #define AFK_VMCNT(n) asm volatile("s_waitcnt vmcnt(" #n ")" ::: "memory")
 #define AFK_LGKMCNT0() asm volatile("s_waitcnt lgkmcnt(0)" ::: "memory")
@@ -79,19 +91,20 @@
     };
 
     const int swz_l = (lane >> 1) & 7;
-    int koffb[4];
-#pragma unroll
-    for (int s = 0; s < 4; ++s) koffb[s] = ((2 * s + hi) ^ swz_l) << 4;
-    const int a_row0 = (wm * 128 + l31) * ROWB;
-    const int b_row0 = OP_BYTES + (wn * 64 + l31) * ROWB;
-
-    f32x16 acc[4][2];
-#pragma unroll
-    for (int i = 0; i < 4; ++i)
-#pragma unroll
-        for (int j = 0; j < 2; ++j)
-#pragma unroll
-            for (int e = 0; e < 16; ++e) acc[i][j][e] = 0.f;
+    const int lrow = lane & (TR - 1), lk = lane / TR;
+    int koffb[NS];
+#pragma unroll
+    for (int s = 0; s < NS; ++s) koffb[s] = (((8 / NS) * s + lk) ^ swz_l) << 4;
+    const int a_row0 = (wm * 128 + lrow) * ROWB;
+    const int b_row0 = OP_BYTES + (wn * 64 + lrow) * ROWB;
+
+    acc_t acc[NI][NJ];
+#pragma unroll
+    for (int i = 0; i < NI; ++i)
+#pragma unroll
+        for (int j = 0; j < NJ; ++j)
+#pragma unroll
+            for (int e = 0; e < NE; ++e) acc[i][j][e] = 0.f;
 
     const int T = p.K / BK;
     issue_x(0);
@@ -105,12 +118,7 @@
     AFK_BARRIER();
     if (wm == 1) AFK_BARRIER();
 
-    bf16x8 bf[2][4], af[2][4];
-#define AFK_MFMA4(ACC0, s)                                                                                         \
-    do {                                                                                                           \
-        _Pragma("unroll") for (int i_ = 0; i_ < 2; ++i_) _Pragma("unroll") for (int j_ = 0; j_ < 2; ++j_)          \
-            acc[ACC0 + i_][j_] = __builtin_amdgcn_mfma_f32_32x32x16_bf16(bf[j_][s], af[i_][s], acc[ACC0 + i_][j_], 0, 0, 0); \
-    } while (0)
+    bf16x8 bf[NJ][NS], af[NI / 2][NS];
     for (int t = 0; t < T; ++t) {
         const char* buf = smem + (t & 1) * BUF_BYTES;
         const int t1 = min(t + 1, T - 1), t2 = min(t + 2, T - 1);
@@ -119,50 +127,64 @@
         char* by = smem + e1 * BUF_BYTES;
         char* bx = smem + e2 * BUF_BYTES;
 #pragma unroll
-        for (int j = 0; j < 2; ++j)
-#pragma unroll
-            for (int s = 0; s < 4; ++s) bf[j][s] = *(const bf16x8*)(buf + b_row0 + j * 32 * ROWB + koffb[s]);
-#pragma unroll
-        for (int i = 0; i < 2; ++i)
-#pragma unroll
-            for (int s = 0; s < 4; ++s) af[i][s] = *(const bf16x8*)(buf + a_row0 + i * 32 * ROWB + koffb[s]);
+        for (int j = 0; j < NJ; ++j)
+#pragma unroll
+            for (int s = 0; s < NS; ++s) bf[j][s] = *(const bf16x8*)(buf + b_row0 + j * TR * ROWB + koffb[s]);
+#pragma unroll
+        for (int i = 0; i < NI / 2; ++i)
+#pragma unroll
+            for (int s = 0; s < NS; ++s) af[i][s] = *(const bf16x8*)(buf + a_row0 + i * TR * ROWB + koffb[s]);
         AFK_LGKMCNT0();
         AFK_VMCNT(6);
         AFK_BARRIER();
         __builtin_amdgcn_s_setprio(1);
-        AFK_MFMA4(0, 0);
-        __builtin_amdgcn_sched_barrier(0);
-        __builtin_amdgcn_global_load_lds((gbl_void*)(ysrc[0] + oy), (lds_void*)(by + ydst[0]), 16, 0, 0);
-        __builtin_amdgcn_sched_barrier(0);
-        AFK_MFMA4(0, 1);
-        __builtin_amdgcn_sched_barrier(0);
-        __builtin_amdgcn_global_load_lds((gbl_void*)(ysrc[1] + oy), (lds_void*)(by + ydst[1]), 16, 0, 0);
-        __builtin_amdgcn_sched_barrier(0);
-        AFK_MFMA4(0, 2);
-        AFK_MFMA4(0, 3);
+#pragma unroll
+        for (int s = 0; s < NS; ++s) {
+#pragma unroll
+            for (int i = 0; i < NI / 2; ++i) {
+#pragma unroll
+                for (int j = 0; j < NJ; ++j) acc[i][j] = AFK_MFMA(bf[j][s], af[i][s], acc[i][j]);
+                const int done = (s * (NI / 2) + i + 1) * NJ;
+                if (done == QSEG || done == 2 * QSEG) {
+                    const int piece = done / QSEG - 1;
+                    __builtin_amdgcn_sched_barrier(0);
+                    __builtin_amdgcn_global_load_lds((gbl_void*)(ysrc[piece] + oy), (lds_void*)(by + ydst[piece]), 16, 0, 0);
+                    __builtin_amdgcn_sched_barrier(0);
+                }
+            }
+        }
         __builtin_amdgcn_s_setprio(0);
         AFK_VMCNT(8);
         AFK_BARRIER();
 #pragma unroll
-        for (int i = 0; i < 2; ++i)
-#pragma unroll
-            for (int s = 0; s < 4; ++s) af[i][s] = *(const bf16x8*)(buf + a_row0 + (i + 2) * 32 * ROWB + koffb[s]);
+        for (int i = 0; i < NI / 2; ++i)
+#pragma unroll
+            for (int s = 0; s < NS; ++s) af[i][s] = *(const bf16x8*)(buf + a_row0 + (i + NI / 2) * TR * ROWB + koffb[s]);
         AFK_LGKMCNT0();
         AFK_VMCNT(2);
         AFK_BARRIER();
         __builtin_amdgcn_s_setprio(1);
 #pragma unroll
-        for (int s = 0; s < 4; ++s) {
-#pragma unroll
-            for (int i = 0; i < 2; ++i) {
-                acc[2 + i][0] = __builtin_amdgcn_mfma_f32_32x32x16_bf16(bf[0][s], af[i][s], acc[2 + i][0], 0, 0, 0);
-                acc[2 + i][1] = __builtin_amdgcn_mfma_f32_32x32x16_bf16(bf[1][s], af[i][s], acc[2 + i][1], 0, 0, 0);
-                const int piece = 2 * s + i;
+        for (int s = 0; s < NS; ++s) {
+#pragma unroll
+            for (int i = 0; i < NI / 2; ++i) {
+#pragma unroll
+                for (int j = 0; j < NJ; ++j) acc[NI / 2 + i][j] = AFK_MFMA(bf[j][s], af[i][s], acc[NI / 2 + i][j]);
+                const int piece = s * (NI / 2) + i;
+#ifdef AFK_DMA_SLOT8
+                if (piece < 6 && (piece & 1)) {
+                    __builtin_amdgcn_sched_barrier(0);
+                    __builtin_amdgcn_global_load_lds((gbl_void*)(xsrc[piece - 1] + ox), (lds_void*)(bx + xdst[piece - 1]), 16, 0, 0);
+                    __builtin_amdgcn_global_load_lds((gbl_void*)(xsrc[piece] + ox), (lds_void*)(bx + xdst[piece]), 16, 0, 0);
+                    __builtin_amdgcn_sched_barrier(0);
+                }
+#else
                 if (piece < 6) {
                     __builtin_amdgcn_sched_barrier(0);
                     __builtin_amdgcn_global_load_lds((gbl_void*)(xsrc[piece] + ox), (lds_void*)(bx + xdst[piece]), 16, 0, 0);
                     __builtin_amdgcn_sched_barrier(0);
                 }
+#endif
             }
         }
         __builtin_amdgcn_s_setprio(0);
@@ -170,9 +192,15 @@
         AFK_BARRIER();
     }
     AFK_VMCNT(0);
-#undef AFK_MFMA4
     if (wm == 0) AFK_BARRIER();
 
+#ifdef AFK_MFMA_16
+#define AFK_PIECE_SWAP(i, j, t, e) \
+    __builtin_amdgcn_permlane16_swap(__float_as_uint(acc[2 * (i)][2 * (j) + (t)][e]), __float_as_uint(acc[2 * (i) + 1][2 * (j) + (t)][e]), false, false)
+#else
+#define AFK_PIECE_SWAP(i, j, t, e) \
+    __builtin_amdgcn_permlane32_swap(__float_as_uint(acc[i][j][8 * (t) + (e)]), __float_as_uint(acc[i][j][8 * (t) + 4 + (e)]), false, false)
+#endif
     if constexpr (EPI == AFK_GEMM_SWIGLU_FWD) {
         typedef __attribute__((ext_vector_type(8))) __bf16 b8;
         const int I = p.N >> 1;
@@ -189,7 +217,7 @@
                     b8 o;
 #pragma unroll
                     for (int e = 0; e < 4; ++e) {
-                        const auto r = __builtin_amdgcn_permlane32_swap(__float_as_uint(acc[i][j][8 * t + e]), __float_as_uint(acc[i][j][8 * t + 4 + e]), false, false);
+                        const auto r = AFK_PIECE_SWAP(i, j, t, e);
                         o[e] = (bf16)(__uint_as_float(r[0]) * p.alpha);
                         o[4 + e] = (bf16)(__uint_as_float(r[1]) * p.alpha);
                     }
@@ -242,7 +270,7 @@
                     b8 o;
 #pragma unroll
                     for (int e = 0; e < 4; ++e) {
-                        const auto r = __builtin_amdgcn_permlane32_swap(__float_as_uint(acc[i][j][8 * t + e]), __float_as_uint(acc[i][j][8 * t + 4 + e]), false, false);
+                        const auto r = AFK_PIECE_SWAP(i, j, t, e);
                         float v0 = __uint_as_float(r[0]) * p.alpha, v1 = __uint_as_float(r[1]) * p.alpha;
                         if constexpr ((EPI & AFK_GEMM_BIAS) != 0) {
                             v0 += (float)bv[e];
@@ -291,7 +319,15 @@
 #pragma unroll
     for (int i = 0; i < 4; ++i)
 #pragma unroll
-        for (int j = 0; j < 2; ++j) gemm_store_block32<EPI>(p, m0 + wm * 128 + i * 32 + l31, n0 + wn * 64 + j * 32, hi, acc[i][j]);
+        for (int j = 0; j < 2; ++j) {
+#ifdef AFK_MFMA_16
+            const GemmBlock16 blk = {{acc[2 * i][2 * j], acc[2 * i][2 * j + 1], acc[2 * i + 1][2 * j], acc[2 * i + 1][2 * j + 1]}};
+            gemm_store_block16<EPI>(p, m0 + wm * 128 + i * 32, n0 + wn * 64 + j * 32, lane, blk);
+#else
+            gemm_store_block32<EPI>(p, m0 + wm * 128 + i * 32 + l31, n0 + wn * 64 + j * 32, hi, acc[i][j]);
+#endif
+        }
+#undef AFK_PIECE_SWAP
 }
 
 }
diff --git a/audio-flamingo_amd/csrc/gemm256t.hip b/audio-flamingo_amd/csrc/gemm256t.hip
--- a/audio-flamingo_amd/csrc/gemm256t.hip
+++ b/audio-flamingo_amd/csrc/gemm256t.hip
@@ -24,19 +24,38 @@
         __builtin_amdgcn_global_load_lds((gbl_void*)(SRCPTR), (lds_void*)(DSTPTR), 16, 0, 0);             \
         __builtin_amdgcn_sched_barrier(0);                                                                \
     } while (0)
+#ifdef AFK_MFMA_16
+constexpr int TR = 16, NI = 8, NJ = 4, NS = 2;
+typedef f32x4 acc_t;
+#define MFMA(a, b, c) __builtin_amdgcn_mfma_f32_16x16x32_bf16(a, b, c, 0, 0, 0)
+#else
+constexpr int TR = 32, NI = 4, NJ = 2, NS = 4;
+typedef f32x16 acc_t;
 #define MFMA(a, b, c) __builtin_amdgcn_mfma_f32_32x32x16_bf16(a, b, c, 0, 0, 0)
+#endif
+constexpr int KS = 64 / NS;
+constexpr int NBA = 2, NAA = 4;
+constexpr int QSEG = (NI / 2) * NJ * NS / 4;
+
+__device__ __forceinline__ int fresh_lane() { return (int)__builtin_amdgcn_mbcnt_hi(~0u, __builtin_amdgcn_mbcnt_lo(~0u, 0u)); }
 
 __device__ __forceinline__ int tswz(int r) { return ((r & 3) << 2) | ((r >> 2) & 3); }
 
-__device__ __forceinline__ int tr_off(int tile32, int pc, int lane) {
-    const int g = lane >> 4, i = lane & 15, hi = g >> 1;
-    const int chunk = 4 * tile32 + 2 * (g & 1) + ((i & 3) >> 1);
+__device__ __forceinline__ int tr_off(int tile, int pc, int lane) {
+    const int g = lane >> 4, i = lane & 15;
+#ifdef AFK_MFMA_16
+    const int chunk = 2 * tile + ((i & 3) >> 1);
+    const int r = 8 * g + (i >> 2) + 4 * pc;
+#else
+    const int hi = g >> 1;
+    const int chunk = 4 * tile + 2 * (g & 1) + ((i & 3) >> 1);
     const int r = 8 * hi + (i >> 2) + 4 * pc;
+#endif
     return r * TROW + ((chunk ^ tswz(r)) << 4) + 8 * (i & 1);
 }
-template <int S>
+template <int S, int FAR = 0>
 __device__ __forceinline__ bf16x8 tr_frag(uint32_t buf, int off0, int off1) {
-    return afk_lds_tr_frag<S * 16 * TROW>(buf + off0, buf + off1);
+    return afk_lds_tr_frag<S * KS * TROW + FAR * 256>(buf + off0, buf + off1);
 }
 
 struct TSrc {
@@ -61,7 +80,7 @@
     const int lane = tid & 63;
     const int wave = __builtin_amdgcn_readfirstlane(tid >> 6);
     const int wm = wave >> 2, wn = wave & 3;
-    const int hi = lane >> 5, l31 = lane & 31;
+    [[maybe_unused]] const int hi = lane >> 5, l31 = lane & 31;
 
     int tm, tn;
     gemm_tile_of_block(p, tm, tn);
@@ -113,20 +132,21 @@
             dst[j] = unit * 1024;
         }
     }
-    const bf16* tbase[NX + NY];
-#pragma unroll
-    for (int j = 0; j < NX + NY; ++j) tbase[j] = (AT || j < 4) ? tr_src[j].base + (int64_t)tr_src[j].krow * tr_ld[j] : nullptr;
-    f32x16 acc[4][2];
-#pragma unroll
-    for (int i = 0; i < 4; ++i)
-#pragma unroll
-        for (int j = 0; j < 2; ++j)
-#pragma unroll
-            for (int e = 0; e < 16; ++e) acc[i][j][e] = 0.f;
+    acc_t acc[NI][NJ];
+#pragma unroll
+    for (int i = 0; i < NI; ++i)
+#pragma unroll
+        for (int j = 0; j < NJ; ++j)
+#pragma unroll
+            for (int e = 0; e < TR * TR / 64; ++e) acc[i][j][e] = 0.f;
 
     const bool ragged = (KL % BK) != 0;
   auto pipeline = [&](auto rag_) {
     constexpr bool RAG = decltype(rag_)::value;
+    const int lane = fresh_lane();
+    const bf16* tbase[NX + NY];
+#pragma unroll
+    for (int j = 0; j < NX + NY; ++j) tbase[j] = (!RAG && (AT || j < 4)) ? tr_src[j].base + (int64_t)tr_src[j].krow * tr_ld[j] : nullptr;
     auto src_of = [&](int j, int t) -> const bf16* {
         const bool tr = AT || j < 4;
         if (tr) {
@@ -141,20 +161,21 @@
     };
     auto issue = [&](int j, int t_src, int parity) { AFK_DMA_PTR(src_of(j, t_src), smem + parity * BUF_BYTES + dst[j]); };
 
-    int tob[2][2], toa[4][2];
-#pragma unroll
-    for (int j = 0; j < 2; ++j)
-#pragma unroll
-        for (int pc = 0; pc < 2; ++pc) tob[j][pc] = OP_BYTES + tr_off(wn * 2 + j, pc, lane);
-#pragma unroll
-    for (int i = 0; i < 4; ++i)
-#pragma unroll
-        for (int pc = 0; pc < 2; ++pc) toa[i][pc] = AT ? tr_off(wm * 4 + i, pc, lane) : 0;
+    int tob[NBA][2], toa[NAA][2];
+#pragma unroll
+    for (int j = 0; j < NBA; ++j)
+#pragma unroll
+        for (int pc = 0; pc < 2; ++pc) tob[j][pc] = OP_BYTES + tr_off(wn * NBA + j, pc, lane);
+#pragma unroll
+    for (int i = 0; i < NAA; ++i)
+#pragma unroll
+        for (int pc = 0; pc < 2; ++pc) toa[i][pc] = AT ? tr_off(wm * NAA + i, pc, lane) : 0;
     const int swz_l = (lane >> 1) & 7;
-    int koffb[4];
-#pragma unroll
-    for (int s = 0; s < 4; ++s) koffb[s] = ((2 * s + hi) ^ swz_l) << 4;
-    const int a_row0 = (wm * 128 + l31) * 128;
+    const int lrow = lane & (TR - 1), lk = lane / TR;
+    int koffb[NS];
+#pragma unroll
+    for (int s = 0; s < NS; ++s) koffb[s] = (((8 / NS) * s + lk) ^ swz_l) << 4;
+    const int a_row0 = (wm * 128 + lrow) * 128;
 
 #pragma unroll
     for (int j = 0; j < NX; ++j) issue(j, 0, 0);
@@ -169,7 +190,7 @@
     AFK_BARRIER();
     if (wm == 1) AFK_BARRIER();
 
-    bf16x8 bf[2][4], af[AT ? 4 : 2][AT ? 2 : 4];
+    bf16x8 bf[NJ][NS], af[AT ? NI : NI / 2][AT ? NS / 2 : NS];
     const uint32_t lds0 = afk_lds_addr(smem);
     for (int t = 0; t < T; ++t) {
         const char* buf = smem + (t & 1) * BUF_BYTES;
@@ -177,43 +198,46 @@
         const int t1 = min(t + 1, T - 1), t2 = min(t + 2, T - 1);
         const int e1 = (t + 1) & 1, e2 = t & 1;
         if (!AT) {
-#pragma unroll
-            for (int j = 0; j < 2; ++j)
-                afk_static_for<4>([&](auto s_) { constexpr int s = decltype(s_)::value; bf[j][s] = tr_frag<s>(lbuf, tob[j][0], tob[j][1]); });
-#pragma unroll
-            for (int i = 0; i < 2; ++i)
-#pragma unroll
-                for (int s = 0; s < 4; ++s) af[i][s] = *(const bf16x8*)(buf + a_row0 + i * 32 * 128 + koffb[s]);
+            afk_static_for<NJ>([&](auto j_) {
+                constexpr int j = decltype(j_)::value;
+                afk_static_for<NS>([&](auto s_) { constexpr int s = decltype(s_)::value; bf[j][s] = tr_frag<s, j / NBA>(lbuf, tob[j % NBA][0], tob[j % NBA][1]); });
+            });
+#pragma unroll
+            for (int i = 0; i < NI / 2; ++i)
+#pragma unroll
+                for (int s = 0; s < NS; ++s) af[i][s] = *(const bf16x8*)(buf + a_row0 + i * TR * 128 + koffb[s]);
             AFK_LGKMCNT0();
             AFK_VMCNT(6);
             AFK_BARRIER();
             __builtin_amdgcn_s_setprio(1);
 #pragma unroll
-            for (int s = 0; s < 4; ++s) {
-#pragma unroll
-                for (int i = 0; i < 2; ++i)
-#pragma unroll
-                    for (int j = 0; j < 2; ++j) acc[i][j] = MFMA(bf[j][s], af[i][s], acc[i][j]);
-                if (s < 2) issue(NX + s, t1, e1);
+            for (int s = 0; s < NS; ++s) {
+#pragma unroll
+                for (int i = 0; i < NI / 2; ++i) {
+#pragma unroll
+                    for (int j = 0; j < NJ; ++j) acc[i][j] = MFMA(bf[j][s], af[i][s], acc[i][j]);
+                    const int done = (s * (NI / 2) + i + 1) * NJ;
+                    if (done == QSEG || done == 2 * QSEG) issue(NX + done / QSEG - 1, t1, e1);
+                }
             }
             __builtin_amdgcn_s_setprio(0);
             AFK_VMCNT(8);
             AFK_BARRIER();
 #pragma unroll
-            for (int i = 0; i < 2; ++i)
-#pragma unroll
-                for (int s = 0; s < 4; ++s) af[i][s] = *(const bf16x8*)(buf + a_row0 + (i + 2) * 32 * 128 + koffb[s]);
+            for (int i = 0; i < NI / 2; ++i)
+#pragma unroll
+                for (int s = 0; s < NS; ++s) af[i][s] = *(const bf16x8*)(buf + a_row0 + (i + NI / 2) * TR * 128 + koffb[s]);
             AFK_LGKMCNT0();
             AFK_VMCNT(2);
             AFK_BARRIER();
             __builtin_amdgcn_s_setprio(1);
 #pragma unroll
-            for (int s = 0; s < 4; ++s) {
-#pragma unroll
-                for (int i = 0; i < 2; ++i) {
-                    acc[2 + i][0] = MFMA(bf[0][s], af[i][s], acc[2 + i][0]);
-                    acc[2 + i][1] = MFMA(bf[1][s], af[i][s], acc[2 + i][1]);
-                    const int piece = 2 * s + i;
+            for (int s = 0; s < NS; ++s) {
+#pragma unroll
+                for (int i = 0; i < NI / 2; ++i) {
+#pragma unroll
+                    for (int j = 0; j < NJ; ++j) acc[NI / 2 + i][j] = MFMA(bf[j][s], af[i][s], acc[NI / 2 + i][j]);
+                    const int piece = s * (NI / 2) + i;
                     if (piece < 6) issue(piece, t2, e2);
                 }
             }
@@ -222,31 +246,31 @@
             AFK_BARRIER();
         } else {
             const int kvalid = KL - t * BK;
+            constexpr int PS = NS / 2;
 #pragma unroll
             for (int ph = 0; ph < 2; ++ph) {
-                afk_static_for<2>([&](auto s_) {
+                afk_static_for<PS>([&](auto s_) {
                     constexpr int s = decltype(s_)::value;
-                    if (ph == 0) {
-#pragma unroll
-                        for (int j = 0; j < 2; ++j) bf[j][s] = tr_frag<s>(lbuf, tob[j][0], tob[j][1]);
-#pragma unroll
-                        for (int i = 0; i < 4; ++i) af[i][s] = tr_frag<s>(lbuf, toa[i][0], toa[i][1]);
-                    } else {
-#pragma unroll
-                        for (int j = 0; j < 2; ++j) bf[j][s] = tr_frag<2 + s>(lbuf, tob[j][0], tob[j][1]);
-#pragma unroll
-                        for (int i = 0; i < 4; ++i) af[i][s] = tr_frag<2 + s>(lbuf, toa[i][0], toa[i][1]);
-                    }
+                    afk_static_for<NJ>([&](auto j_) {
+                        constexpr int j = decltype(j_)::value;
+                        if (ph == 0) bf[j][s] = tr_frag<s, j / NBA>(lbuf, tob[j % NBA][0], tob[j % NBA][1]);
+                        else bf[j][s] = tr_frag<PS + s, j / NBA>(lbuf, tob[j % NBA][0], tob[j % NBA][1]);
+                    });
+                    afk_static_for<NI>([&](auto i_) {
+                        constexpr int i = decltype(i_)::value;
+                        if (ph == 0) af[i][s] = tr_frag<s, i / NAA>(lbuf, toa[i % NAA][0], toa[i % NAA][1]);
+                        else af[i][s] = tr_frag<PS + s, i / NAA>(lbuf, toa[i % NAA][0], toa[i % NAA][1]);
+                    });
                 });
                 AFK_LGKMCNT0();
                 if (RAG && kvalid < BK) {
 #pragma unroll
-                    for (int s = 0; s < 2; ++s)
+                    for (int s = 0; s < PS; ++s)
 #pragma unroll
                         for (int e = 0; e < 8; ++e) {
-                            const bool dead = 16 * (2 * ph + s) + 8 * hi + e >= kvalid;
-#pragma unroll
-                            for (int i = 0; i < 4; ++i)
+                            const bool dead = KS * (PS * ph + s) + 8 * lk + e >= kvalid;
+#pragma unroll
+                            for (int i = 0; i < NI; ++i)
                                 if (dead) af[i][s][e] = (bf16)0.f;
                         }
                 }
@@ -254,12 +278,12 @@
                 AFK_BARRIER();
                 __builtin_amdgcn_s_setprio(1);
 #pragma unroll
-                for (int s = 0; s < 2; ++s) {
-#pragma unroll
-                    for (int i = 0; i < 4; ++i) {
-                        acc[i][0] = MFMA(bf[0][s], af[i][s], acc[i][0]);
-                        acc[i][1] = MFMA(bf[1][s], af[i][s], acc[i][1]);
-                        const int piece = 4 * s + i;
+                for (int s = 0; s < PS; ++s) {
+#pragma unroll
+                    for (int i = 0; i < NI; ++i) {
+#pragma unroll
+                        for (int j = 0; j < NJ; ++j) acc[i][j] = MFMA(bf[j][s], af[i][s], acc[i][j]);
+                        const int piece = NI * s + i;
                         if ((piece & 1) == 0) {
                             if (ph == 0) issue(NX + (piece >> 1), t1, e1);
                             else issue(piece >> 1, t2, e2);
@@ -281,7 +305,15 @@
 #pragma unroll
     for (int i = 0; i < 4; ++i)
 #pragma unroll
-        for (int j = 0; j < 2; ++j) gemm_store_block32<EPI>(p, m0 + wm * 128 + i * 32 + l31, n0 + wn * 64 + j * 32, hi, acc[i][j]);
+        for (int j = 0; j < 2; ++j) {
+#ifdef AFK_MFMA_16
+            const GemmBlock16 blk = {{acc[2 * i][2 * j], acc[2 * i][2 * j + 1], acc[2 * i + 1][2 * j], acc[2 * i + 1][2 * j + 1]}};
+            const int mb = AT ? m0 + wm * 64 + (i & 1) * 32 + (i >> 1) * 128 : m0 + wm * 128 + i * 32;
+            gemm_store_block16<EPI>(p, mb, n0 + wn * 32 + j * 128, fresh_lane(), blk);
+#else
+            gemm_store_block32<EPI>(p, m0 + wm * 128 + i * 32 + l31, n0 + wn * 64 + j * 32, hi, acc[i][j]);
+#endif
+        }
 }
 
 }
diff --git a/audio-flamingo_amd/csrc/gemm_common.h b/audio-flamingo_amd/csrc/gemm_common.h
--- a/audio-flamingo_amd/csrc/gemm_common.h
+++ b/audio-flamingo_amd/csrc/gemm_common.h
@@ -35,6 +35,10 @@
 #define AFK_GM_RAW(p) false
 #endif
 
+#ifndef AFK_MFMA_32
+#define AFK_MFMA_16 1
+#endif
+
 typedef __attribute__((address_space(3))) void lds_void;
 typedef const __attribute__((address_space(1))) void gbl_void;
 
@@ -172,6 +176,70 @@
     }
 }
 
+struct GemmBlock16 {
+    f32x4 c[4];
+};
+__device__ __forceinline__ void gemm_block16_gather8(const f32x4& top, const f32x4& bot, float v[8]) {
+#pragma unroll
+    for (int e = 0; e < 4; ++e) {
+        const auto r = __builtin_amdgcn_permlane16_swap(__float_as_uint(top[e]), __float_as_uint(bot[e]), false, false);
+        v[e] = __uint_as_float(r[0]);
+        v[4 + e] = __uint_as_float(r[1]);
+    }
+}
+template <int F>
+__device__ __forceinline__ void gemm_store_block16_body(const GemmArgs& p, int mb, int nb, int lane, const GemmBlock16& b) {
+    const int r = lane & 15, g = lane >> 4;
+    if (F == -2 || (F == -1 && p.splits > 1)) {
+#pragma unroll
+        for (int ii = 0; ii < 2; ++ii)
+#pragma unroll
+            for (int jj = 0; jj < 2; ++jj) {
+                const int m = mb + 16 * ii + r, n = nb + 16 * jj + 4 * g;
+                if (m < p.M && n < p.N) *(f32x4*)(p.ws + ((int64_t)blockIdx.y * p.M + m) * p.N + n) = b.c[2 * ii + jj];
+            }
+        return;
+    }
+    if constexpr (F == -2) return;
+    if (F >= 0 || p.wide) {
+#pragma unroll
+        for (int t = 0; t < 2; ++t) {
+            float v[8];
+            gemm_block16_gather8(b.c[t], b.c[2 + t], v);
+            const int m = mb + (lane & 31), n = nb + 16 * t + 8 * (lane >> 5);
+            if (m < p.M && n < p.N) gemm_epilogue_store<8, F>(p, m, n, v);
+        }
+        return;
+    }
+#pragma unroll
+    for (int ii = 0; ii < 2; ++ii)
+#pragma unroll
+        for (int jj = 0; jj < 2; ++jj) {
+            const int m = mb + 16 * ii + r, n = nb + 16 * jj + 4 * g;
+            if (m >= p.M || n >= p.N) continue;
+            const f32x4& c = b.c[2 * ii + jj];
+            float v[4] = {c[0], c[1], c[2], c[3]};
+            gemm_epilogue_store<4, F>(p, m, n, v);
+        }
+}
+static __device__ __noinline__ void gemm_store_block16_generic(const GemmArgs& p, int mb, int nb, int lane, f32x16 v) {
+    GemmBlock16 b;
+#pragma unroll
+    for (int q = 0; q < 4; ++q) b.c[q] = f32x4{v[4 * q], v[4 * q + 1], v[4 * q + 2], v[4 * q + 3]};
+    gemm_store_block16_body<-1>(p, mb, nb, lane, b);
+}
+template <int F = -1>
+__device__ __forceinline__ void gemm_store_block16(const GemmArgs& p, int mb, int nb, int lane, const GemmBlock16& b) {
+    if constexpr (F == -1) {
+        f32x16 v;
+#pragma unroll
+        for (int q = 0; q < 16; ++q) v[q] = b.c[q >> 2][q & 3];
+        gemm_store_block16_generic(p, mb, nb, lane, v);
+    } else {
+        gemm_store_block16_body<F>(p, mb, nb, lane, b);
+    }
+}
+
 int afk_launch_gemm256(const GemmArgs& p, hipStream_t st);
 int afk_launch_gemm256p(const GemmArgs& p, hipStream_t st);
 int afk_launch_gemm256q(const GemmArgs& p, hipStream_t st);
```

Result: faster. 651.7 audio-s/s, median of 6 (+2.9%).
